# 666DZY666/micronet

Measured on NVIDIA H100. Metric: qat_step_images_per_sec, higher is better.
Workload: dtype f32 (bf16 tensor-core products of exact integer levels / exact bf16 pieces, fp32 accumulate)

## Files before the change

### include/micronet_b200.h

```cpp
#ifndef MICRONET_B200_H
#define MICRONET_B200_H

#include <stdint.h>

#ifdef __cplusplus
extern "C" {
#endif

typedef void* mnb_stream_t;

#define MNB_E_ARG (-1)
#define MNB_E_UNSUPPORTED (-2)

int mnb_version(void);
const char* mnb_last_error(void);
int64_t mnb_launch_count(void);

typedef struct {
  int32_t batch, in_c, in_h, in_w;
  int32_t out_c, ker_h, ker_w;
  int32_t stride_h, stride_w, pad_h, pad_w, dil_h, dil_w, groups;
} mnb_conv_shape;

#define MNB_ACT_DOREFA 1
#define MNB_ACT_IAO 2
#define MNB_ACT_SIGN 3

typedef struct {
  int32_t mode;
  int32_t bits;
  int32_t qmin, qmax;
  int32_t q_type;
  const float* scale;
  const float* zero_point;
  const float* obs_min;
  const float* obs_max;
} mnb_act_qparams;

int mnb_act_quant_fwd(const float* x, int64_t n, const mnb_act_qparams* qp, uint8_t* codes,
                      uint32_t* pass_bits, float* xq, mnb_stream_t stream);
int mnb_act_quant_bwd(const float* g, const uint32_t* pass_bits, int64_t n, const mnb_act_qparams* qp,
                      float* dx, mnb_stream_t stream);

int mnb_bn_fold_fwd(const float* w, int32_t out_c, int32_t per_channel, const float* gamma, const float* beta,
                    const float* bias, const float* mean, const float* var, double eps, float* w_fused, float* b_fused,
                    mnb_stream_t stream);
int mnb_bn_fold_bwd(const float* dw_fused, const float* db_fused, const float* w, int32_t out_c, int32_t per_channel,
                    const float* gamma, const float* bias, const float* mean, const float* var, double eps, float* dw,
                    float* out6, mnb_stream_t stream);
int mnb_bn_fold_running(float* running_mean, float* running_var, const float* batch_mean, const float* batch_var, int32_t n,
                        double momentum, int32_t first, mnb_stream_t stream);

int mnb_quant_add_fwd(const float* a, const float* b, int64_t n, const mnb_act_qparams* qp, float* out,
                      uint32_t* pass_bits_a, uint32_t* pass_bits_b, int32_t relu ,
                      mnb_stream_t stream);
int mnb_quant_add_bwd(const float* g, const uint32_t* pass_bits_a, const uint32_t* pass_bits_b, int64_t n,
                      const mnb_act_qparams* qp, float* da, float* db, mnb_stream_t stream);

int64_t mnb_observe_scratch_bytes(int64_t n, int32_t rows);
int mnb_iao_observe(const float* x, int64_t n, int32_t rows, int32_t observer_kind, int32_t first,
                    double momentum, double percentile, float* min_val, float* max_val,
                    int32_t update_qparams, int32_t symmetric, int32_t qmin, int32_t qmax,
                    float* scale, float* zero_point, void* scratch, mnb_stream_t stream);
int mnb_iao_update_qparams(const float* min_val, const float* max_val, int32_t rows, int32_t symmetric,
                           int32_t qmin, int32_t qmax, float* scale, float* zero_point,
                           mnb_stream_t stream);

int mnb_dorefa_weight_fwd(const float* w, int64_t numel, int32_t out_c, int32_t w_bits, int16_t* w_int,
                          float* w_scale, float* wq, float* aux, void* scratch, mnb_stream_t stream);
int mnb_dorefa_weight_bwd(const float* g_wq, const float* aux, int64_t numel, int32_t w_bits, float* dw,
                          void* scratch, mnb_stream_t stream);
int mnb_wb_weight_fwd(float* w, int32_t out_c, int32_t in_c_per_group, int32_t ker_hw, int32_t W,
                      int16_t* w_int, float* w_scale, float* wq, float* aux, mnb_stream_t stream);
int mnb_wb_weight_bwd(const float* g_wq, const float* w, const float* aux, int32_t out_c,
                      int32_t in_c_per_group, int32_t ker_hw, int32_t W, float* dw, mnb_stream_t stream);
int mnb_iao_weight_fwd(const float* w, int64_t numel, int32_t out_c, int32_t rows, const float* scale,
                       const float* zero_point, const float* obs_min, const float* obs_max,
                       int32_t q_type, int32_t qmin, int32_t qmax, int16_t* w_int, float* w_scale,
                       float* wq, uint8_t* pass, mnb_stream_t stream);
int mnb_iao_weight_bwd(const float* g_wq, const uint8_t* pass, const float* scale, int64_t numel,
                       int32_t out_c, int32_t rows, float* dw, mnb_stream_t stream);

typedef struct {
  const uint8_t* a_codes;
  const float* a_f32;
  int32_t a_offset;
  const float* a_offset_zp;
  const float* a_scale;
  const int16_t* w_int;
  const float* w_scale;
  const float* w_f32;
  const float* bias;
} mnb_conv_operands;

int mnb_conv2d_fwd(const mnb_conv_shape* s, const mnb_conv_operands* op, float* y, mnb_stream_t stream);
int mnb_conv2d_dgrad(const mnb_conv_shape* s, const float* dy, const float* wq, const uint32_t* pass_bits,
                     const mnb_act_qparams* qp, float* dx, mnb_stream_t stream);
int64_t mnb_wgrad_scratch_bytes(const mnb_conv_shape* s);
int mnb_conv2d_wgrad(const mnb_conv_shape* s, const float* dy, const mnb_conv_operands* op, float* dwq,
                     void* scratch, mnb_stream_t stream);
int mnb_channel_stats(const float* x, int32_t batch, int32_t channels, int32_t hw, int32_t as_mean_var,
                      float* stats, void* scratch, mnb_stream_t stream);
int mnb_channel_stats_bwd(const float* x, const float* mean, const float* dmean, const float* dvar,
                          int32_t batch, int32_t channels, int32_t hw, float* dx, mnb_stream_t stream);

int mnb_fq_conv2d_fwd_tc(const mnb_conv_shape* s, const float* x, const mnb_act_qparams* qp,
                         const int16_t* w_int, const float* w_scale, const float* bias, float* y,
                         uint8_t* codes, uint32_t* pass_bits, void* wpack_scratch, int32_t* err_flag,
                         mnb_stream_t stream);

int mnb_conv2d_dgrad_tc(const mnb_conv_shape* s, const float* dy, const int16_t* w_int, const float* w_scale,
                        const uint32_t* pass_bits, const mnb_act_qparams* qp, float* dx, void* wpack_scratch,
                        int32_t* err_flag, mnb_stream_t stream);

int64_t mnb_wgrad_tc_scratch_bytes(const mnb_conv_shape* s);
int mnb_conv2d_wgrad_tc(const mnb_conv_shape* s, const float* dy, const float* x, const mnb_act_qparams* qp,
                        float* dwq, void* scratch, int32_t* inexact_flag, int32_t* err_flag, mnb_stream_t stream);
int mnb_conv2d_wgrad_cond(const mnb_conv_shape* s, const float* dy, const mnb_conv_operands* op, float* dwq,
                          void* scratch, const int32_t* run_if_nonzero, mnb_stream_t stream);

int mnb_bn_batch_stats(const float* x, int32_t batch, int32_t channels, int32_t hw, double eps, double momentum,
                       float* running_mean, float* running_var, int64_t* num_batches_tracked, float* mean_invstd,
                       void* scratch, mnb_stream_t stream);
int mnb_bn_sign_fwd(const float* x, int32_t batch, int32_t channels, int32_t hw, const float* mean, const float* invstd,
                    const float* gamma, const float* beta, int32_t out_shuffle_groups, float* y, uint32_t* pass_bits,
                    mnb_stream_t stream);
int mnb_bn_sign_bwd(const float* g, const uint32_t* pass_bits, const float* x, int32_t batch, int32_t channels, int32_t hw,
                    const float* mean, const float* invstd, const float* gamma, int32_t training,
                    int32_t out_shuffle_groups, float* dx, float* dgamma, float* dbeta, float* dx_channel_sum,
                    void* scratch, mnb_stream_t stream);

int mnb_bn_sign_pool_fwd(const float* x, int32_t batch, int32_t channels, int32_t H, int32_t W, const float* mean,
                         const float* invstd, const float* gamma, const float* beta, int32_t out_shuffle_groups, float* y,
                         uint32_t* pass_bits, uint8_t* argmax, mnb_stream_t stream);
int mnb_bn_sign_pool_bwd(const float* g, const uint32_t* pass_bits, const uint8_t* argmax, const float* x, int32_t batch,
                         int32_t channels, int32_t H, int32_t W, const float* mean, const float* invstd, const float* gamma,
                         int32_t training, int32_t out_shuffle_groups, float* dx, float* dgamma, float* dbeta,
                         float* dx_channel_sum, void* scratch, mnb_stream_t stream);

int mnb_maxpool2d_fwd(const float* x, int32_t batch, int32_t channels, int32_t H, int32_t W, int32_t kernel, int32_t stride,
                      int32_t pad, int32_t out_shuffle_groups, float* y, uint8_t* argmax, mnb_stream_t stream);
int mnb_maxpool2d_bwd(const float* g, const uint8_t* argmax, int32_t batch, int32_t channels, int32_t H, int32_t W,
                      int32_t kernel, int32_t stride, int32_t pad, int32_t out_shuffle_groups, float* dx,
                      mnb_stream_t stream);

int mnb_bn_sign_fwd_packed(const float* x, int32_t batch, int32_t channels, int32_t hw, const float* mean,
                           const float* invstd, const float* gamma, const float* beta, int32_t out_shuffle_groups, float* y,
                           uint32_t* pass_bits, void* x_packed, mnb_stream_t stream);

int mnb_fconv2d_fwd_tc(const mnb_conv_shape* s, const float* x, const float* w, const float* bias, float* y,
                       int32_t* err_flag, mnb_stream_t stream);
int64_t mnb_fconv2d_wgrad_tc_scratch_bytes(const mnb_conv_shape* s);
int mnb_fconv2d_wgrad_tc(const mnb_conv_shape* s, const float* dy, const float* x, float* dw, void* scratch,
                         int32_t* err_flag, mnb_stream_t stream);

int64_t mnb_pk_act_bytes(int32_t batch, int32_t channels, int32_t h, int32_t w, int32_t terms);
int mnb_pk_pack_act(const float* x, int32_t batch, int32_t channels, int32_t h, int32_t w, const mnb_act_qparams* qp,
                    int32_t terms, const float* ch_scale, int32_t phase_split, void* out_pk, uint8_t* bits8,
                    mnb_stream_t stream);
int mnb_bn_relu_quant_pack_fwd(const float* x, int32_t batch, int32_t channels, int32_t hw, const float* mean,
                               const float* invstd, const float* gamma, const float* beta, const mnb_act_qparams* qp,
                               int32_t out_shuffle_groups, void* x_packed, uint32_t* pass_bits, mnb_stream_t stream);
int mnb_bn_sign_bwd_pack(const float* g, const uint32_t* pass_bits, const float* x, int32_t batch, int32_t channels, int32_t hw,
                         const float* mean, const float* invstd, const float* gamma, const float* dgamma, const float* dbeta,
                         int32_t out_shuffle_groups, const float* ch_scale, int32_t terms, float* dx, void* dy_packed,
                         mnb_stream_t stream);
int mnb_bn_sign_pool_bwd_pack(const float* g, const uint32_t* pass_bits, const uint8_t* argmax, const float* x, int32_t batch,
                              int32_t channels, int32_t H, int32_t W, const float* mean, const float* invstd,
                              const float* gamma, const float* dgamma, const float* dbeta, int32_t out_shuffle_groups,
                              const float* ch_scale, int32_t terms, void* dy_packed, mnb_stream_t stream);
int mnb_pk_conv_codes(const mnb_conv_shape* s, const void* a_pk, int32_t terms_a, const void* w_img, int32_t terms_w,
                      const float* n_scale, const float* a_scale, float a_scale_const, const float* bias, int32_t level_bound,
                      int16_t* codes, float* dec, int32_t* err_flag, mnb_stream_t stream);
int mnb_codes_decode(const int16_t* codes, const float* dec, int32_t batch, int32_t channels, int32_t hw, float* x,
                     mnb_stream_t stream);
int mnb_bn_batch_stats_codes(const int16_t* codes, const float* dec, int32_t batch, int32_t channels, int32_t hw, double eps,
                             double momentum, float* running_mean, float* running_var, int64_t* num_batches_tracked,
                             float* mean_invstd, void* scratch, mnb_stream_t stream);
int mnb_bn_sign_fwd_packed_codes(const int16_t* codes, const float* dec, int32_t batch, int32_t channels, int32_t hw,
                                 const float* mean, const float* invstd, const float* gamma, const float* beta,
                                 int32_t out_shuffle_groups, float* y, uint32_t* pass_bits, void* x_packed, mnb_stream_t stream);
int mnb_bn_sign_bwd_codes(const float* g, const uint32_t* pass_bits, const int16_t* codes, const float* dec, int32_t batch,
                          int32_t channels, int32_t hw, const float* mean, const float* invstd, const float* gamma,
                          int32_t training, int32_t out_shuffle_groups, float* dx, float* dgamma, float* dbeta,
                          float* dx_channel_sum, void* scratch, mnb_stream_t stream);
int mnb_bn_sign_pool_fwd_codes(const int16_t* codes, const float* dec, int32_t batch, int32_t channels, int32_t H, int32_t W,
                               const float* mean, const float* invstd, const float* gamma, const float* beta,
                               int32_t out_shuffle_groups, float* y, uint32_t* pass_bits, uint8_t* argmax, mnb_stream_t stream);
int mnb_bn_sign_pool_bwd_codes(const float* g, const uint32_t* pass_bits, const uint8_t* argmax, const int16_t* codes,
                               const float* dec, int32_t batch, int32_t channels, int32_t H, int32_t W, const float* mean,
                               const float* invstd, const float* gamma, int32_t training, int32_t out_shuffle_groups, float* dx,
                               float* dgamma, float* dbeta, float* dx_channel_sum, void* scratch, mnb_stream_t stream);
int mnb_bn_sign_bwd_pack_codes(const float* g, const uint32_t* pass_bits, const int16_t* codes, const float* dec, int32_t batch,
                               int32_t channels, int32_t hw, const float* mean, const float* invstd, const float* gamma,
                               const float* dgamma, const float* dbeta, int32_t out_shuffle_groups, const float* ch_scale,
                               int32_t terms, float* dx, void* dy_packed, mnb_stream_t stream);
int mnb_bn_sign_pool_bwd_pack_codes(const float* g, const uint32_t* pass_bits, const uint8_t* argmax, const int16_t* codes,
                                    const float* dec, int32_t batch, int32_t channels, int32_t H, int32_t W, const float* mean,
                                    const float* invstd, const float* gamma, const float* dgamma, const float* dbeta,
                                    int32_t out_shuffle_groups, const float* ch_scale, int32_t terms, void* dy_packed,
                                    mnb_stream_t stream);
int mnb_pk_pack_act_relu(const float* x, int32_t batch, int32_t channels, int32_t h, int32_t w, const mnb_act_qparams* qp,
                         int32_t terms, const float* ch_scale, int32_t phase_split, int32_t relu, void* out_pk,
                         uint8_t* bits8, mnb_stream_t stream);
int mnb_pk_conv_plan(const mnb_conv_shape* s, int32_t mode, int32_t terms_a, int32_t terms_w, int32_t* out16);
int mnb_pk_conv_plan_ex(const mnb_conv_shape* s, int32_t mode, int32_t terms_a, int32_t terms_w, int32_t* out, int32_t n);
int mnb_pk_wgrad_plan(const mnb_conv_shape* s, int32_t terms_dy, int32_t terms_x, int32_t* out, int32_t n);
int64_t mnb_pk_wimage_bytes(const mnb_conv_shape* s, int32_t mode, int32_t terms_a, int32_t terms_w);
int mnb_pk_pack_weight(const mnb_conv_shape* s, int32_t mode, int32_t terms_a, int32_t terms_w, const int16_t* w_int,
                       const float* w_f32, const float* kzero, void* w_img, mnb_stream_t stream);
int mnb_pk_conv(const mnb_conv_shape* s, int32_t mode, const void* a_pk, int32_t terms_a, const void* w_img, int32_t terms_w,
                const float* n_scale, const float* a_scale, float a_scale_const, const float* bias, const uint8_t* bits8,
                float gain, float* out, int32_t* err_flag, mnb_stream_t stream);
typedef struct mnb_pk_post {
  const mnb_act_qparams* q;
  int32_t relu;
  int32_t phase_split;
  void* out_pk;
} mnb_pk_post;
int mnb_pk_conv_post(const mnb_conv_shape* s, const void* a_pk, int32_t terms_a, const void* w_img, int32_t terms_w,
                     const float* n_scale, const float* a_scale, float a_scale_const, const float* bias, float* out,
                     const mnb_pk_post* post, int32_t* err_flag, mnb_stream_t stream);
int mnb_quant_add_pack_fwd(const float* a, const float* b, int32_t batch, int32_t channels, int32_t h, int32_t w,
                           const mnb_act_qparams* qp, int32_t relu, float* out, const mnb_pk_post* post, mnb_stream_t stream);
int64_t mnb_pk_i8_act_bytes(int32_t batch, int32_t channels, int32_t h, int32_t w);
int mnb_pk_i8_pack_act(const float* x, int32_t batch, int32_t channels, int32_t h, int32_t w, const mnb_act_qparams* qp,
                       int32_t phase_split, int32_t relu, void* out_pk, mnb_stream_t stream);
int mnb_pk_i8_conv_plan(const mnb_conv_shape* s, int32_t* out, int32_t n);
int64_t mnb_pk_i8_wimage_bytes(const mnb_conv_shape* s);
int mnb_pk_i8_pack_weight(const mnb_conv_shape* s, const int16_t* w_int, void* w_img, mnb_stream_t stream);
int mnb_pk_i8_conv(const mnb_conv_shape* s, const void* a_pk, const void* w_img, const float* n_scale, const float* a_scale,
                   float a_scale_const, const float* bias, float* out, const mnb_pk_post* post, int32_t* err_flag,
                   mnb_stream_t stream);
int mnb_quant_add_pack_i8_fwd(const float* a, const float* b, int32_t batch, int32_t channels, int32_t h, int32_t w,
                              const mnb_act_qparams* qp, int32_t relu, float* out, const mnb_pk_post* post, mnb_stream_t stream);
int64_t mnb_pk_wgrad_scratch_bytes(const mnb_conv_shape* s, int32_t terms_dy, int32_t terms_x);
int mnb_pk_wgrad(const mnb_conv_shape* s, const void* dy_pk, int32_t terms_dy, const void* x_pk, int32_t terms_x,
                 const float* a_scale, const float* kdiv, float* dw, void* scratch, int32_t* err_flag, mnb_stream_t stream);
int mnb_pk_wgrad_taps_plan(const mnb_conv_shape* s, int32_t terms_dy, int32_t terms_x, int32_t* out, int32_t n);
int mnb_pk_wgrad_taps(const mnb_conv_shape* s, const void* dy_pk, int32_t terms_dy, const void* x_pk, int32_t terms_x,
                      const float* a_scale, const float* kdiv, float* dw, void* scratch, int32_t* err_flag, mnb_stream_t stream);

int mnb_xnor_supported(const mnb_conv_shape* s);
int64_t mnb_xnor_act_bytes(int32_t batch, int32_t channels, int32_t h, int32_t w, int32_t groups);
int mnb_xnor_pack_act(const float* x, int32_t batch, int32_t channels, int32_t h, int32_t w, int32_t groups, void* out_bits,
                      mnb_stream_t stream);
int64_t mnb_xnor_wimage_bytes(const mnb_conv_shape* s);
int mnb_xnor_pack_weight(const mnb_conv_shape* s, const int16_t* w_int, void* w_img, mnb_stream_t stream);
int mnb_xnor_conv_fwd(const mnb_conv_shape* s, const void* a_bits, const void* w_img, const float* alpha, const float* bias,
                      float* y, mnb_stream_t stream);

int mnb_adam_step(float* params, const float* grads, float* exp_avg, float* exp_avg_sq, int64_t n, float lr,
                  float beta1, float beta2, float eps, float weight_decay, int32_t step, mnb_stream_t stream);

void mnb_set_tc_profile_buffer(void* dev_int64x16);

int mnb_selftest_umma(const float* A, const float* B, float* D, int32_t N, int32_t K, int32_t int8,
                      int32_t* err_flag, mnb_stream_t stream);
int mnb_selftest_tma3d(const float* src, const int64_t* dims3_host, const int32_t* box3_host,
                       const int32_t* coord3_host, float* out, int32_t* err_flag, mnb_stream_t stream);

int mnb_selftest_mma_rate(int32_t N, int32_t n_acc, int32_t a_shift16, int32_t iters, int32_t mn_major,
                          int64_t* out2, int32_t* err_flag, mnb_stream_t stream);

#ifdef __cplusplus
}
#endif
#endif
```

### micronet_b200/_lib.py

```python
from __future__ import annotations

import ctypes as C
import os

import torch

_HERE = os.path.dirname(os.path.abspath(__file__))
LIB_PATH = os.path.join(_HERE, "lib", "libmicronet_b200.so")

ACT_DOREFA, ACT_IAO, ACT_SIGN = 1, 2, 3


class ConvShape(C.Structure):
    _fields_ = [(n, C.c_int32) for n in (
        "batch", "in_c", "in_h", "in_w", "out_c", "ker_h", "ker_w", "stride_h", "stride_w",
        "pad_h", "pad_w", "dil_h", "dil_w", "groups")]


class ActQParams(C.Structure):
    _fields_ = [("mode", C.c_int32), ("bits", C.c_int32), ("qmin", C.c_int32), ("qmax", C.c_int32),
                ("q_type", C.c_int32), ("scale", C.c_void_p), ("zero_point", C.c_void_p),
                ("obs_min", C.c_void_p), ("obs_max", C.c_void_p)]


class PkPost(C.Structure):
    _fields_ = [("q", C.POINTER(ActQParams)), ("relu", C.c_int32), ("phase_split", C.c_int32), ("out_pk", C.c_void_p)]


class ConvOperands(C.Structure):
    _fields_ = [("a_codes", C.c_void_p), ("a_f32", C.c_void_p), ("a_offset", C.c_int32),
                ("a_offset_zp", C.c_void_p), ("a_scale", C.c_void_p), ("w_int", C.c_void_p),
                ("w_scale", C.c_void_p), ("w_f32", C.c_void_p), ("bias", C.c_void_p)]


_P, _I, _L, _D = C.c_void_p, C.c_int32, C.c_int64, C.c_double
_SHAPE, _ACTQ, _OPS = C.POINTER(ConvShape), C.POINTER(ActQParams), C.POINTER(ConvOperands)

PROTOTYPES = {
    "mnb_version": (C.c_int, []),
    "mnb_last_error": (C.c_char_p, []),
    "mnb_launch_count": (_L, []),
    "mnb_act_quant_fwd": (C.c_int, [_P, _L, _ACTQ, _P, _P, _P, _P]),
    "mnb_act_quant_bwd": (C.c_int, [_P, _P, _L, _ACTQ, _P, _P]),
    "mnb_bn_fold_fwd": (C.c_int, [_P, _I, _I, _P, _P, _P, _P, _P, _D, _P, _P, _P]),
    "mnb_bn_fold_bwd": (C.c_int, [_P, _P, _P, _I, _I, _P, _P, _P, _P, _D, _P, _P, _P]),
    "mnb_bn_fold_running": (C.c_int, [_P, _P, _P, _P, _I, _D, _I, _P]),
    "mnb_quant_add_fwd": (C.c_int, [_P, _P, _L, _ACTQ, _P, _P, _P, _I, _P]),
    "mnb_quant_add_bwd": (C.c_int, [_P, _P, _P, _L, _ACTQ, _P, _P, _P]),
    "mnb_observe_scratch_bytes": (_L, [_L, _I]),
    "mnb_iao_observe": (C.c_int, [_P, _L, _I, _I, _I, _D, _D, _P, _P, _I, _I, _I, _I, _P, _P, _P, _P]),
    "mnb_iao_update_qparams": (C.c_int, [_P, _P, _I, _I, _I, _I, _P, _P, _P]),
    "mnb_dorefa_weight_fwd": (C.c_int, [_P, _L, _I, _I, _P, _P, _P, _P, _P, _P]),
    "mnb_dorefa_weight_bwd": (C.c_int, [_P, _P, _L, _I, _P, _P, _P]),
    "mnb_wb_weight_fwd": (C.c_int, [_P, _I, _I, _I, _I, _P, _P, _P, _P, _P]),
    "mnb_wb_weight_bwd": (C.c_int, [_P, _P, _P, _I, _I, _I, _I, _P, _P]),
    "mnb_iao_weight_fwd": (C.c_int, [_P, _L, _I, _I, _P, _P, _P, _P, _I, _I, _I, _P, _P, _P, _P, _P]),
    "mnb_iao_weight_bwd": (C.c_int, [_P, _P, _P, _L, _I, _I, _P, _P]),
    "mnb_conv2d_fwd": (C.c_int, [_SHAPE, _OPS, _P, _P]),
    "mnb_conv2d_dgrad": (C.c_int, [_SHAPE, _P, _P, _P, _ACTQ, _P, _P]),
    "mnb_wgrad_scratch_bytes": (_L, [_SHAPE]),
    "mnb_conv2d_wgrad": (C.c_int, [_SHAPE, _P, _OPS, _P, _P, _P]),
    "mnb_channel_stats": (C.c_int, [_P, _I, _I, _I, _I, _P, _P, _P]),
    "mnb_channel_stats_bwd": (C.c_int, [_P, _P, _P, _P, _I, _I, _I, _P, _P]),
    "mnb_fq_conv2d_fwd_tc": (C.c_int, [_SHAPE, _P, _ACTQ, _P, _P, _P, _P, _P, _P, _P, _P, _P]),
    "mnb_conv2d_dgrad_tc": (C.c_int, [_SHAPE, _P, _P, _P, _P, _ACTQ, _P, _P, _P, _P]),
    "mnb_wgrad_tc_scratch_bytes": (_L, [_SHAPE]),
    "mnb_conv2d_wgrad_tc": (C.c_int, [_SHAPE, _P, _P, _ACTQ, _P, _P, _P, _P, _P]),
    "mnb_conv2d_wgrad_cond": (C.c_int, [_SHAPE, _P, _OPS, _P, _P, _P, _P]),
    "mnb_bn_batch_stats": (C.c_int, [_P, _I, _I, _I, _D, _D, _P, _P, _P, _P, _P, _P]),
    "mnb_bn_sign_fwd": (C.c_int, [_P, _I, _I, _I, _P, _P, _P, _P, _I, _P, _P, _P]),
    "mnb_bn_sign_bwd": (C.c_int, [_P, _P, _P, _I, _I, _I, _P, _P, _P, _I, _I, _P, _P, _P, _P, _P, _P]),
    "mnb_bn_sign_pool_fwd": (C.c_int, [_P, _I, _I, _I, _I, _P, _P, _P, _P, _I, _P, _P, _P, _P]),
    "mnb_bn_sign_pool_bwd": (C.c_int, [_P, _P, _P, _P, _I, _I, _I, _I, _P, _P, _P, _I, _I, _P, _P, _P, _P, _P, _P]),
    "mnb_bn_sign_fwd_packed": (C.c_int, [_P, _I, _I, _I, _P, _P, _P, _P, _I, _P, _P, _P, _P]),
    "mnb_fconv2d_fwd_tc": (C.c_int, [_SHAPE, _P, _P, _P, _P, _P, _P]),
    "mnb_fconv2d_wgrad_tc_scratch_bytes": (_L, [_SHAPE]),
    "mnb_fconv2d_wgrad_tc": (C.c_int, [_SHAPE, _P, _P, _P, _P, _P, _P]),
    "mnb_maxpool2d_fwd": (C.c_int, [_P, _I, _I, _I, _I, _I, _I, _I, _I, _P, _P, _P]),
    "mnb_maxpool2d_bwd": (C.c_int, [_P, _P, _I, _I, _I, _I, _I, _I, _I, _I, _P, _P]),
    "mnb_adam_step": (C.c_int, [_P, _P, _P, _P, _L, C.c_float, C.c_float, C.c_float, C.c_float, C.c_float, _I, _P]),
    "mnb_pk_act_bytes": (_L, [_I, _I, _I, _I, _I]),
    "mnb_pk_pack_act": (C.c_int, [_P, _I, _I, _I, _I, _ACTQ, _I, _P, _I, _P, _P, _P]),
    "mnb_bn_relu_quant_pack_fwd": (C.c_int, [_P, _I, _I, _I, _P, _P, _P, _P, _ACTQ, _I, _P, _P, _P]),
    "mnb_pk_pack_act_relu": (C.c_int, [_P, _I, _I, _I, _I, _ACTQ, _I, _P, _I, _I, _P, _P, _P]),
    "mnb_pk_conv_plan": (C.c_int, [_SHAPE, _I, _I, _I, _P]),
    "mnb_pk_conv_plan_ex": (C.c_int, [_SHAPE, _I, _I, _I, _P, _I]),
    "mnb_pk_wgrad_plan": (C.c_int, [_SHAPE, _I, _I, _P, _I]),
    "mnb_pk_wimage_bytes": (_L, [_SHAPE, _I, _I, _I]),
    "mnb_pk_pack_weight": (C.c_int, [_SHAPE, _I, _I, _I, _P, _P, _P, _P, _P]),
    "mnb_pk_conv": (C.c_int, [_SHAPE, _I, _P, _I, _P, _I, _P, _P, C.c_float, _P, _P, C.c_float, _P, _P, _P]),
    "mnb_bn_sign_bwd_pack": (C.c_int, [_P, _P, _P, _I, _I, _I, _P, _P, _P, _P, _P, _I, _P, _I, _P, _P, _P]),
    "mnb_bn_sign_pool_bwd_pack": (C.c_int, [_P, _P, _P, _P, _I, _I, _I, _I, _P, _P, _P, _P, _P, _I, _P, _I, _P, _P]),
    "mnb_pk_conv_post": (C.c_int, [_SHAPE, _P, _I, _P, _I, _P, _P, C.c_float, _P, _P, C.POINTER(PkPost), _P, _P]),
    "mnb_pk_conv_codes": (C.c_int, [_SHAPE, _P, _I, _P, _I, _P, _P, C.c_float, _P, _I, _P, _P, _P, _P]),
    "mnb_codes_decode": (C.c_int, [_P, _P, _I, _I, _I, _P, _P]),
    "mnb_bn_batch_stats_codes": (C.c_int, [_P, _P, _I, _I, _I, _D, _D, _P, _P, _P, _P, _P, _P]),
    "mnb_bn_sign_fwd_packed_codes": (C.c_int, [_P, _P, _I, _I, _I, _P, _P, _P, _P, _I, _P, _P, _P, _P]),
    "mnb_bn_sign_bwd_codes": (C.c_int, [_P, _P, _P, _P, _I, _I, _I, _P, _P, _P, _I, _I, _P, _P, _P, _P, _P, _P]),
    "mnb_bn_sign_pool_fwd_codes": (C.c_int, [_P, _P, _I, _I, _I, _I, _P, _P, _P, _P, _I, _P, _P, _P, _P]),
    "mnb_bn_sign_pool_bwd_codes": (C.c_int, [_P, _P, _P, _P, _P, _I, _I, _I, _I, _P, _P, _P, _I, _I, _P, _P, _P, _P, _P, _P]),
    "mnb_bn_sign_bwd_pack_codes": (C.c_int, [_P, _P, _P, _P, _I, _I, _I, _P, _P, _P, _P, _P, _I, _P, _I, _P, _P, _P]),
    "mnb_bn_sign_pool_bwd_pack_codes": (C.c_int, [_P, _P, _P, _P, _P, _I, _I, _I, _I, _P, _P, _P, _P, _P, _I, _P, _I, _P,
                                                  _P]),
    "mnb_quant_add_pack_fwd": (C.c_int, [_P, _P, _I, _I, _I, _I, _ACTQ, _I, _P, C.POINTER(PkPost), _P]),
    "mnb_pk_i8_act_bytes": (_L, [_I, _I, _I, _I]),
    "mnb_pk_i8_pack_act": (C.c_int, [_P, _I, _I, _I, _I, _ACTQ, _I, _I, _P, _P]),
    "mnb_pk_i8_conv_plan": (C.c_int, [_SHAPE, _P, _I]),
    "mnb_pk_i8_wimage_bytes": (_L, [_SHAPE]),
    "mnb_pk_i8_pack_weight": (C.c_int, [_SHAPE, _P, _P, _P]),
    "mnb_pk_i8_conv": (C.c_int, [_SHAPE, _P, _P, _P, _P, C.c_float, _P, _P, C.POINTER(PkPost), _P, _P]),
    "mnb_quant_add_pack_i8_fwd": (C.c_int, [_P, _P, _I, _I, _I, _I, _ACTQ, _I, _P, C.POINTER(PkPost), _P]),
    "mnb_pk_wgrad_scratch_bytes": (_L, [_SHAPE, _I, _I]),
    "mnb_pk_wgrad": (C.c_int, [_SHAPE, _P, _I, _P, _I, _P, _P, _P, _P, _P, _P]),
    "mnb_pk_wgrad_taps_plan": (C.c_int, [_SHAPE, _I, _I, _P, _I]),
    "mnb_pk_wgrad_taps": (C.c_int, [_SHAPE, _P, _I, _P, _I, _P, _P, _P, _P, _P, _P]),
    "mnb_xnor_supported": (C.c_int, [_SHAPE]),
    "mnb_xnor_act_bytes": (_L, [_I, _I, _I, _I, _I]),
    "mnb_xnor_pack_act": (C.c_int, [_P, _I, _I, _I, _I, _I, _P, _P]),
    "mnb_xnor_wimage_bytes": (_L, [_SHAPE]),
    "mnb_xnor_pack_weight": (C.c_int, [_SHAPE, _P, _P, _P]),
    "mnb_xnor_conv_fwd": (C.c_int, [_SHAPE, _P, _P, _P, _P, _P, _P]),
    "mnb_set_tc_profile_buffer": (None, [_P]),
    "mnb_selftest_mma_rate": (C.c_int, [_I, _I, _I, _I, _I, _P, _P, _P]),
    "mnb_selftest_umma": (C.c_int, [_P, _P, _P, _I, _I, _I, _P, _P]),
    "mnb_selftest_tma3d": (C.c_int, [_P, C.POINTER(C.c_int64), C.POINTER(C.c_int32), C.POINTER(C.c_int32), _P, _P, _P]),
}

_lib = None


def load():
    global _lib
    if _lib is not None:
        return _lib
    if not os.path.exists(LIB_PATH):
        raise RuntimeError(
            f"micronet_b200: {LIB_PATH} is missing - build it with `python -m micronet_b200.build` "
            "(there is no CPU / PyTorch fallback for the fake-quant hot path)")
    lib = C.CDLL(LIB_PATH)
    for name, (res, args) in PROTOTYPES.items():
        fn = getattr(lib, name)
        fn.restype, fn.argtypes = res, args
    _lib = lib
    return lib


def check(rc: int, what: str):
    if rc != 0:
        msg = load().mnb_last_error().decode(errors="replace")
        kind = ValueError if rc < 0 else RuntimeError
        raise kind(f"micronet_b200.{what} failed (code {rc}): {msg}")


def ptr(t):
    return None if t is None else t.data_ptr()


def stream():
    return torch.cuda.current_stream().cuda_stream


def require_cuda(*tensors):
    for t in tensors:
        if t is not None and not t.is_cuda:
            raise RuntimeError(
                "micronet_b200: the fake-quant engine runs on CUDA (sm_90a) tensors only; "
                "got a CPU tensor - there is deliberately no CPU fallback")


def require_f32(*tensors):
    for t in tensors:
        if t is not None and t.dtype != torch.float32:
            raise TypeError(f"micronet_b200: fp32 tensors only (the reference's QAT modules are fp32), got {t.dtype}")


def launch_count() -> int:
    return int(load().mnb_launch_count())


_errflags = {}


def tc_err_flag(device):
    key = (device.type, device.index)
    if key not in _errflags:
        _errflags[key] = torch.zeros(1, dtype=torch.int32, device=device)
    return _errflags[key]


def tc_check(device=None):
    for key, flag in _errflags.items():
        code = int(flag.item())
        if code:
            raise RuntimeError(f"micronet_b200: tensor-core pipeline wait timed out (code {code}) on {key}")


E_UNSUPPORTED = -2
KEEP_DEBUG = False
USE_TC = os.environ.get("MNB_DISABLE_TC", "0") != "1"
USE_PACKED = os.environ.get("MNB_PACKED_OPERANDS", "0") == "1"
PK_MODE = os.environ.get("MNB_PK", "auto")
PK_TERMS = int(os.environ.get("MNB_PK_TERMS", "3"))
PK_TERMS_BWD = int(os.environ.get("MNB_PK_TERMS_BWD", "2"))
PK_WBWTAB = os.environ.get("MNB_PK_WBWTAB", "1") == "1"
PK_WG_TAPS = os.environ.get("MNB_PK_WG_TAPS", "1") != "0"

XNOR_MODE = os.environ.get("MNB_XNOR", "auto")

PLANE_ONLY = os.environ.get("MNB_PLANE_ONLY", "1") == "1"

_scratch = {}


def scratch(device, rows=1):
    lib = load()
    need = int(lib.mnb_observe_scratch_bytes(0, int(rows)))
    key = (device.type, device.index)
    buf = _scratch.get(key)
    if buf is None or buf.numel() < need:
        buf = torch.zeros(max(need, 1 << 20), dtype=torch.uint8, device=device)
        _scratch[key] = buf
    return buf
```

### micronet_b200/csrc/mnb_pk.cu

```cuda
#include <cuda.h>
#include <cuda_bf16.h>

#include <algorithm>
#include <cstdlib>
#include <cstring>

#include "mnb_common.cuh"
#include "mnb_tc.cuh"

namespace pk {

constexpr int MAXST = 8;
constexpr int MAXTAP = 64, MAXTMPL = 16, MAXY = 4, MAXPAIR = 6, MAXPROG = 512;
constexpr int kSmemBudget = 227 * 1024 - 3072;
constexpr int kNtSizes[] = {16, 32, 48, 64, 96, 128};

struct Tmpl { int kph, tap0, ntap, blk_off, blk_bytes; };

struct Plan {
  int mode;
  int B, G, R, S, stride;
  int HA, WA, C8A, nkph;
  int kg, ng, NOUT;
  int OHr, OWr, OH, OW, omul, ny;
  int hlo, hhi, wlo, whi;
  int Wt, BW, TH, THH, TB, npos, col_tiles, row_tiles, img_tiles, n_mtiles;
  int Nt, n_ntiles, MT, n_mgroups, n_items;
  int CC, ksteps, chunks;
  int TA, TBk, npairs, pair_a[MAXPAIR], pair_b[MAXPAIR];
  int ntmpl[MAXY], ntap[MAXY];
  Tmpl tmpl[MAXY][MAXTMPL];
  int tap_aoff[MAXY][MAXTAP];
  short tap_r[MAXY][MAXTAP], tap_s[MAXY][MAXTAP];
  int img_bytes[MAXY], y_off[MAXY];
  int64_t wimg_bytes;
  int a_box_bytes, a_bytes, b_off, stage_bytes, nstage, st_log2, smem_bytes, off_stg;
  int segmented, seg_len;
  int cpu;
};

static inline int ceil_div(int a, int b) { return (a + b - 1) / b; }
static inline int round_up(int a, int b) { return ceil_div(a, b) * b; }

static void make_pairs(int TA, int TBk, Plan& p) {
  const int lim = std::max(TA, TBk) - 1;
  p.npairs = 0;
  for (int sum = lim; sum >= 0; --sum)
    for (int a = 0; a < TA; ++a) {
      const int b = sum - a;
      if (b < 0 || b >= TBk) continue;
      if (p.npairs < MAXPAIR) { p.pair_a[p.npairs] = a; p.pair_b[p.npairs] = b; ++p.npairs; }
    }
}

static int unsupported(const char* why) { return mnb_fail(MNB_E_UNSUPPORTED, "pk conv: %s", why); }

static int make_plan(const mnb_conv_shape* s, int mode, int TA, int TBk, Plan& p, int cpu = 8) {
  MNB_REQUIRE(s != nullptr, "conv shape is NULL");
  memset(&p, 0, sizeof(p));
  const int C = s->in_c, K = s->out_c, G = s->groups, H = s->in_h, W = s->in_w, R = s->ker_h, S = s->ker_w;
  MNB_REQUIRE(s->batch > 0 && C > 0 && K > 0 && H > 0 && W > 0 && G > 0 && C % G == 0 && K % G == 0 && R > 0 && S > 0,
              "bad conv shape");
  MNB_REQUIRE(TA >= 1 && TA <= 3 && TBk >= 1 && TBk <= 3, "term counts must be 1..3");
  MNB_REQUIRE(cpu == 8 || (cpu == 16 && mode == 0 && TA == 1 && TBk == 1), "int8 plans are single-product forward plans");
  if (s->dil_h != 1 || s->dil_w != 1) return unsupported("dilation != 1");
  if (s->stride_h != s->stride_w || (s->stride_h != 1 && s->stride_h != 2)) return unsupported("stride must be 1 or 2");
  const int st = s->stride_h, ph_ = s->pad_h, pw_ = s->pad_w;
  if (ph_ > R - 1 || pw_ > S - 1) return unsupported("padding larger than the filter");
  const int P = (H + 2 * ph_ - R) / st + 1, Q = (W + 2 * pw_ - S) / st + 1;
  if (P < 1 || Q < 1) return unsupported("empty output");
  if (st == 2 && ((H | W) & 1)) return unsupported("stride 2 needs even H and W");
  const int cin_g = C / G, cout_g = K / G;
  p.mode = mode; p.B = s->batch; p.G = G; p.R = R; p.S = S; p.stride = st;
  p.TA = TA; p.TBk = TBk; p.cpu = cpu;
  make_pairs(TA, TBk, p);
  if (mode == 0) {
    p.kg = cin_g; p.ng = cout_g; p.NOUT = K;
    p.nkph = st == 2 ? 4 : 1;
    p.HA = H / st; p.WA = W / st; p.C8A = ceil_div(C, cpu);
    p.OHr = P; p.OWr = Q; p.OH = P; p.OW = Q; p.omul = 1; p.ny = 1;
  } else {
    p.kg = cout_g; p.ng = cin_g; p.NOUT = C;
    p.nkph = 1; p.HA = P; p.WA = Q; p.C8A = ceil_div(K, 8);
    p.OHr = H / st; p.OWr = W / st; p.OH = H; p.OW = W; p.omul = st; p.ny = st == 2 ? 4 : 1;
  }
  if (G > 1 && (p.kg % cpu))
    return unsupported(cpu == 8 ? "grouped conv needs GEMM-K channels per group % 8 == 0"
                                : "grouped int8 conv needs GEMM-K channels per group % 16 == 0");
  if (cpu == 16 && (int64_t)p.kg * R * S * 128 * 127 > (int64_t)INT32_MAX) return unsupported("int8 sums could overflow s32");
  struct Tap { int kph, sh, sw, r, s; };
  Tap taps[MAXY][MAXTAP];
  int hlo = 0, hhi = 0, wlo = 0, whi = 0;
  for (int y = 0; y < p.ny; ++y) {
    int n = 0;
    const int ya = y >> 1, yb = y & 1;
    for (int kph = 0; kph < p.nkph; ++kph)
      for (int r = 0; r < R; ++r)
        for (int q = 0; q < S; ++q) {
          int kp = 0, sh, sw;
          if (mode == 0) {
            const int dr = r - ph_, ds = q - pw_;
            if (st == 1) { sh = dr; sw = ds; }
            else {
              const int fh = dr & 1, fw = ds & 1;
              kp = fh * 2 + fw; sh = (dr - fh) / 2; sw = (ds - fw) / 2;
            }
          } else {
            if (st == 1) { sh = ph_ - r; sw = pw_ - q; }
            else {
              const int th = ya + ph_ - r, tw = yb + pw_ - q;
              if ((th & 1) || (tw & 1)) continue;
              sh = th / 2; sw = tw / 2;
            }
          }
          if (kp != kph) continue;
          if (n >= MAXTAP) return unsupported("more than 64 filter taps");
          taps[y][n++] = Tap{kph, sh, sw, r, q};
          hlo = std::max(hlo, -sh); hhi = std::max(hhi, sh); wlo = std::max(wlo, -sw); whi = std::max(whi, sw);
        }
    p.ntap[y] = n;
  }
  p.hlo = hlo; p.hhi = hhi; p.wlo = wlo; p.whi = whi;
  const int halo_w = wlo + whi;
  if (halo_w >= 96) return unsupported("filter too wide");
  {
    const int ct_min = ceil_div(p.OWr, 128 - halo_w);
    double best = 1e30;
    int ct_max = std::min(p.OWr, ct_min + 14);
    if (p.npairs > 1) {
      const int wt0 = ceil_div(p.OWr, ct_min), bw0 = wt0 + halo_w;
      const int th0 = std::max(1, std::min(p.OHr, (128 - wt0) / bw0 + 1));
      if ((double)((th0 + hlo + hhi) * bw0) / (double)(th0 * wt0) <= 2.2) ct_max = ct_min;
    }
    for (int ct = ct_min; ct <= ct_max; ++ct) {
      const int wt = ceil_div(p.OWr, ct), bw = wt + halo_w;
      if (ceil_div(p.OWr, wt) != ct) continue;
      const int th = std::max(1, std::min(p.OHr, (128 - wt) / bw + 1));
      const double amp = (double)((th + hlo + hhi) * bw) / (double)(th * wt);
      const double cost = (double)ct * ceil_div(p.OHr, th) * (1.0 + 0.25 * amp) * (1.0 + 3.2 / wt);
      if (cost < best - 1e-9) { best = cost; p.col_tiles = ct; p.Wt = wt; p.BW = bw; p.TH = th; }
    }
    if (const char* e = getenv("MNB_PK_COLTILES")) {
      const int ct = atoi(e);
      if (ct >= ct_min && ct <= p.OWr) {
        p.col_tiles = ct; p.Wt = ceil_div(p.OWr, ct); p.col_tiles = ceil_div(p.OWr, p.Wt); p.BW = p.Wt + halo_w;
        p.TH = std::max(1, std::min(p.OHr, (128 - p.Wt) / p.BW + 1));
      }
    }
  }
  p.THH = p.TH + hlo + hhi;
  p.TB = 1;
  if (p.TH == p.OHr && p.col_tiles == 1) {
    const int last = (p.TH - 1) * p.BW + p.Wt;
    p.TB = std::max(1, std::min(p.B, (128 - last) / (p.THH * p.BW) + 1));
  }
  if (p.BW > 128 || p.THH > 256 || p.TB > 256) return unsupported("box dimension");
  p.npos = p.TB * p.THH * p.BW;
  p.row_tiles = ceil_div(p.OHr, p.TH);
  p.img_tiles = ceil_div(p.B, p.TB);
  p.n_mtiles = p.img_tiles * p.row_tiles * p.col_tiles;
  const int ng16 = round_up(p.ng, 16);
  {
    int seg_target = 64;
    if (const char* e = getenv("MNB_PK_SEG_MMAS")) seg_target = std::max(1, atoi(e));
    int chain = 0;
    for (int y = 0; y < p.ny; ++y) chain = std::max(chain, p.ntap[y] * p.npairs * ceil_div(p.kg, 16));
    p.segmented = p.npairs > 1 && chain > seg_target;
  }
  {
    const int ntiles = ceil_div(ng16, 128);
    const int want = round_up(ceil_div(ng16, ntiles), 16);
    p.Nt = 128;
    for (int v : kNtSizes) if (v >= want) { p.Nt = v; break; }
  }
  p.n_ntiles = ceil_div(p.ng, p.Nt);
  p.MT = 1;
  {
    auto wave_eff = [&](int mt) {
      const int64_t items = (int64_t)ceil_div(p.n_mtiles, mt) * p.n_ntiles * G;
      const int64_t ctas = std::max<int64_t>(1, MNB_NUM_SMS / p.ny);
      return (double)items / (double)(ceil_div((int)std::min<int64_t>(items, 1 << 30), (int)ctas) * ctas);
    };
    const int cap = std::max(1, 128 / p.Nt);
    for (int mt = 2; mt <= std::min(4, cap); mt *= 2) {
      if (p.n_mtiles < mt) break;
      if ((int64_t)ceil_div(p.n_mtiles, mt) * p.n_ntiles * G * p.ny < 120) break;
      if (wave_eff(mt) >= wave_eff(1) - 0.04) p.MT = mt;
    }
  }
  if (const char* e = getenv("MNB_PK_MT")) {
    const int v = atoi(e);
    if ((v == 1 || v == 2 || v == 4) && v * p.Nt <= 128) p.MT = v;
  }
  p.n_mgroups = ceil_div(p.n_mtiles, p.MT);
  p.n_items = p.n_mgroups * p.n_ntiles * G;
  const int nk16 = ceil_div(p.kg, 2 * cpu);
  int maxtap_kph = 1;
  for (int y = 0; y < p.ny; ++y)
    for (int i = 0, run = 0; i < p.ntap[y]; ++i) {
      run = (i > 0 && taps[y][i].kph == taps[y][i - 1].kph) ? run + 1 : 1;
      maxtap_kph = std::max(maxtap_kph, run);
    }
  const int a16 = p.MT * TA * round_up(2 * p.npos * 16, 128);
  auto b16 = [&](int tg) { return TBk * tg * 2 * p.Nt * 16; };
  const int stage_target = 56 * 1024;
  int TG = std::min(maxtap_kph, 25);
  while (TG > 1 && a16 + b16(TG) > stage_target) --TG;
  if (a16 + b16(TG) > (kSmemBudget - 8192) / 2) return unsupported("one 16-channel stage does not fit in shared memory");
  int cc16 = std::max(1, std::min(nk16, stage_target / (a16 + b16(TG))));
  cc16 = std::min(cc16, 16);
  p.chunks = ceil_div(nk16, cc16);
  cc16 = ceil_div(nk16, p.chunks);
  p.CC = cc16 * 2 * cpu; p.ksteps = cc16;
  p.a_box_bytes = (p.CC / cpu) * p.npos * 16;
  p.a_bytes = round_up(p.a_box_bytes, 128);
  p.b_off = p.MT * TA * p.a_bytes;
  int64_t total = 0;
  int max_blk = 0;
  for (int y = 0; y < p.ny; ++y) {
    int nt = 0, off = 0;
    for (int i = 0; i < p.ntap[y];) {
      int j = i;
      while (j < p.ntap[y] && taps[y][j].kph == taps[y][i].kph && j - i < TG) ++j;
      if (nt >= MAXTMPL) return unsupported("too many tap groups");
      Tmpl& t = p.tmpl[y][nt++];
      t.kph = taps[y][i].kph; t.tap0 = i; t.ntap = j - i;
      t.blk_bytes = TBk * t.ntap * (p.CC / cpu) * p.Nt * 16;
      t.blk_off = off;
      off += p.chunks * t.blk_bytes;
      max_blk = std::max(max_blk, t.blk_bytes);
      i = j;
    }
    p.ntmpl[y] = nt;
    p.img_bytes[y] = off;
    p.y_off[y] = (int)total;
    total += (int64_t)off * p.n_ntiles * G;
    if (total > (int64_t)1 << 30) return unsupported("weight image larger than 1 GiB");
    for (int i = 0; i < p.ntap[y]; ++i) {
      p.tap_aoff[y][i] = (taps[y][i].sh + hlo) * p.BW + (taps[y][i].sw + wlo);
      p.tap_r[y][i] = (short)taps[y][i].r; p.tap_s[y][i] = (short)taps[y][i].s;
    }
  }
  p.wimg_bytes = std::max<int64_t>(total, 16);
  p.seg_len = 1 << 30;
  if (p.segmented) {
    const int per_stage = TG * p.npairs * p.ksteps;
    int target = 64;
    if (const char* e = getenv("MNB_PK_SEG_MMAS")) target = std::max(1, atoi(e));
    p.seg_len = std::max(1, target / per_stage);
  }
  p.stage_bytes = round_up(p.b_off + max_blk, 1024);
  const int slack = round_up((128 + (hlo + hhi) * p.BW + halo_w + 8) * 16, 1024);
  const int stg = 32 * tc::kStageLd * 4;
  int nst = (kSmemBudget - slack - stg) / p.stage_bytes;
  if (nst < 2) return unsupported("fewer than two pipeline stages fit");
  p.nstage = nst >= 8 ? 8 : (nst >= 4 ? 4 : 2);
  if (const char* e = getenv("MNB_PK_STAGES")) { const int v = atoi(e); if ((v == 2 || v == 4 || v == 8) && v <= nst) p.nstage = v; }
  p.st_log2 = p.nstage == 8 ? 3 : (p.nstage == 4 ? 2 : 1);
  p.off_stg = p.nstage * p.stage_bytes + slack;
  p.smem_bytes = p.off_stg + stg;
  if (p.MT * p.Nt > 128) return unsupported("accumulators exceed the register budget");
  return 0;
}

__device__ __forceinline__ uint32_t pack2(float a, float b) {
  __nv_bfloat162 v = __floats2bfloat162_rn(a, b);
  return *reinterpret_cast<uint32_t*>(&v);
}

__device__ __forceinline__ uint32_t pack4_s8(float a, float b, float c, float d) {
  return ((uint32_t)__float2int_rn(a) & 0xffu) | (((uint32_t)__float2int_rn(b) & 0xffu) << 8) |
         (((uint32_t)__float2int_rn(c) & 0xffu) << 16) | ((uint32_t)__float2int_rn(d) << 24);
}
__device__ __forceinline__ uint4 pack16_s8(const float (&l)[16]) {
  return make_uint4(pack4_s8(l[0], l[1], l[2], l[3]), pack4_s8(l[4], l[5], l[6], l[7]), pack4_s8(l[8], l[9], l[10], l[11]),
                    pack4_s8(l[12], l[13], l[14], l[15]));
}

template <int QUANT>
__global__ void __launch_bounds__(256) pack_act_kernel(const float* __restrict__ x, int B, int C, int H, int W, int C8,
                                                       int terms, const float* __restrict__ ch_scale, mnb_act_qparams qp,
                                                       int a_off, int phase_split, uint4* __restrict__ out,
                                                       int64_t plane_vecs, uint8_t* __restrict__ bits8, int relu) {
  MnbActQ q;
  float zp = 0.f;
  if (QUANT) {
    q = mnb_load_actq(qp);
    if (qp.mode == MNB_ACT_IAO && qp.zero_point) zp = __ldg(qp.zero_point);
  }
  const uint32_t HW = (uint32_t)H * (uint32_t)W;
  const uint32_t plane = blockIdx.y * blockDim.y + threadIdx.y;
  if (plane >= (uint32_t)B * (uint32_t)C8) return;
  const uint32_t b = plane / (uint32_t)C8, c8 = plane - b * (uint32_t)C8;
  for (uint32_t pos = blockIdx.x * blockDim.x + threadIdx.x; pos < HW; pos += gridDim.x * blockDim.x) {
    const int64_t idx = (int64_t)plane * HW + pos;
    float v[8];
    uint32_t passbits = 0;
    const float* src = x + ((int64_t)b * C + c8 * 8) * HW + pos;
#pragma unroll
    for (int j = 0; j < 8; ++j) {
      const int c = (int)c8 * 8 + j;
      float val = c < C ? __ldg(src + (int64_t)j * HW) : 0.f;
      if (relu) val = fmaxf(val, 0.f);
      if (!QUANT && ch_scale) val = c < C ? __fmul_rn(val, __ldg(ch_scale + c)) : 0.f;
      v[j] = val;
    }
    if (QUANT) {
      float lev[8];
      mnb_act_levels<8>(q, v, lev, passbits);
      uint32_t live = 0;
#pragma unroll
      for (int j = 0; j < 8; ++j) {
        const bool in = (int)c8 * 8 + j < C;
        v[j] = in ? lev[j] + zp : 0.f;
        live |= in ? (1u << j) : 0u;
      }
      passbits &= live;
    }
    int64_t dst;
    if (phase_split) {
      const uint32_t h = pos / (uint32_t)W, w = pos - h * (uint32_t)W;
      const uint32_t oct = ((h & 1u) * 2u + (w & 1u)) * (uint32_t)C8 + c8;
      dst = (((int64_t)b * 4 * C8 + oct) * (H >> 1) + (h >> 1)) * (W >> 1) + (w >> 1);
    } else {
      dst = idx;
    }
    for (int tm = 0; tm < terms; ++tm) {
      uint32_t pk4[4];
#pragma unroll
      for (int j = 0; j < 4; ++j) {
        pk4[j] = pack2(v[2 * j], v[2 * j + 1]);
        v[2 * j] -= __uint_as_float(pk4[j] << 16);
        v[2 * j + 1] -= __uint_as_float(pk4[j] & 0xffff0000u);
      }
      out[(int64_t)tm * plane_vecs + dst] = make_uint4(pk4[0], pk4[1], pk4[2], pk4[3]);
    }
    if (QUANT && bits8) bits8[idx] = (uint8_t)passbits;
  }
}

__global__ void __launch_bounds__(256) pack_act_i8_kernel(const float* __restrict__ x, int B, int C, int H, int W, int C16,
                                                          mnb_act_qparams qp, int phase_split, int relu, uint4* __restrict__ out) {
  const MnbActQ q = mnb_load_actq(qp);
  const float zp = qp.zero_point ? __ldg(qp.zero_point) : 0.f;
  const uint32_t HW = (uint32_t)H * (uint32_t)W;
  const uint32_t plane = blockIdx.y * blockDim.y + threadIdx.y;
  if (plane >= (uint32_t)B * (uint32_t)C16) return;
  const uint32_t b = plane / (uint32_t)C16, c16 = plane - b * (uint32_t)C16;
  for (uint32_t pos = blockIdx.x * blockDim.x + threadIdx.x; pos < HW; pos += gridDim.x * blockDim.x) {
    const float* src = x + ((int64_t)b * C + c16 * 16) * HW + pos;
    float v[16], lev[16];
#pragma unroll
    for (int j = 0; j < 16; ++j) {
      float val = (int)c16 * 16 + j < C ? __ldg(src + (int64_t)j * HW) : 0.f;
      if (relu) val = fmaxf(val, 0.f);
      v[j] = val;
    }
    uint32_t passbits;
    mnb_act_levels<16>(q, v, lev, passbits);
#pragma unroll
    for (int j = 0; j < 16; ++j) lev[j] = (int)c16 * 16 + j < C ? lev[j] + zp : 0.f;
    int64_t dst;
    if (phase_split) {
      const uint32_t h = pos / (uint32_t)W, w = pos - h * (uint32_t)W;
      const uint32_t u = ((h & 1u) * 2u + (w & 1u)) * (uint32_t)C16 + c16;
      dst = (((int64_t)b * 4 * C16 + u) * (H >> 1) + (h >> 1)) * (W >> 1) + (w >> 1);
    } else {
      dst = (int64_t)plane * HW + pos;
    }
    out[dst] = pack16_s8(lev);
  }
}

__global__ void __launch_bounds__(256) bn_relu_quant_pack_kernel(const float* __restrict__ x, int batch, int channels, int hw,
                                                                 int sg, const float* __restrict__ mean,
                                                                 const float* __restrict__ invstd, const float* __restrict__ gamma,
                                                                 const float* __restrict__ beta, mnb_act_qparams qp,
                                                                 uint32_t* __restrict__ bits, uint4* __restrict__ xp) {
  const int lane = threadIdx.x & 31;
  const int c8n = channels / 8, p32n = hw / 32, cpg = channels / sg;
  const int64_t items = (int64_t)batch * c8n * p32n;
  const int64_t nwarps = ((int64_t)gridDim.x * blockDim.x) >> 5;
  const MnbActQ q = mnb_load_actq(qp);
  for (int64_t w = ((int64_t)blockIdx.x * blockDim.x + threadIdx.x) >> 5; w < items; w += nwarps) {
    const int p32 = (int)(w % p32n);
    const int64_t t = w / p32n;
    const int oc8 = (int)(t % c8n), b = (int)(t / c8n);
    const int pos = p32 * 32 + lane;
    float lev[8], yv[8], bnv[8];
#pragma unroll
    for (int j = 0; j < 8; ++j) {
      const int oc = oc8 * 8 + j;
      const int c = sg > 1 ? (oc % sg) * cpg + oc / sg : oc;
      const int64_t fi = ((int64_t)b * channels + c) * hw + pos;
      bnv[j] = fmaf(__ldg(x + fi) - __ldg(mean + c), __ldg(gamma + c) * __ldg(invstd + c), __ldg(beta + c));
      yv[j] = fmaxf(bnv[j], 0.f);
    }
    uint32_t passbits;
    mnb_act_levels<8>(q, yv, lev, passbits);
#pragma unroll
    for (int j = 0; j < 8; ++j) {
      const int oc = oc8 * 8 + j;
      const int c = sg > 1 ? (oc % sg) * cpg + oc / sg : oc;
      const int64_t fi = ((int64_t)b * channels + c) * hw + pos;
      const uint32_t word = __ballot_sync(0xffffffffu, ((passbits >> j) & 1u) && bnv[j] > 0.f);
      if (lane == 0) bits[fi >> 5] = word;
    }
    xp[((int64_t)b * c8n + oc8) * hw + pos] = make_uint4(pack2(lev[0], lev[1]), pack2(lev[2], lev[3]), pack2(lev[4], lev[5]),
                                                          pack2(lev[6], lev[7]));
  }
}

template <int CPU>
__global__ void __launch_bounds__(256) quant_add_pack_kernel(const float* __restrict__ a, const float* __restrict__ b, int B, int C,
// ... 419 lines not shown
#pragma unroll
            for (int mt = 0; mt < MAXMT; ++mt) {
              if (mt >= (int)p.m.MT) break;
              const uint32_t a_base = a_lo0 + s16 + (uint32_t)mt * p.m.a_mt16, b_base = b_lo0 + s16;
              for (uint32_t e = 0; e < pc; ++e) {
                const uint4 w4 = p.m.prog4[pb + e];
                const uint32_t w[4] = {w4.x, w4.y, w4.z, w4.w};
#pragma unroll
                for (int k = 0; k < 4; ++k) {
                  if (w[k] == 0xffffffffu) continue;
                  if constexpr (I8)
                    tc::Mma<NT>::s8(reinterpret_cast<int32_t(&)[NR]>(acc[mt]), a_hi | (uint64_t)(a_base + (w[k] & 0xffffu)),
                                    b_hi | (uint64_t)(b_base + (w[k] >> 16)), 1);
                  else
                    tc::Mma<NT>::template bf16<0, 0>(acc[mt], a_hi | (uint64_t)(a_base + (w[k] & 0xffffu)),
                                                      b_hi | (uint64_t)(b_base + (w[k] >> 16)), 1);
                }
              }
            }
          }
          tc::wg_commit();
          tc::wg_wait<0>();
#pragma unroll
          for (int mt = 0; mt < MAXMT; ++mt) tc::fence_acc(acc[mt]);
          __syncwarp();
          if (lane == 0) tc::mbar_arrive(&sh.empty[slot]);
          if (SEG && ++seg_pos == p.m.seg_len) {
            seg_pos = 0;
#pragma unroll
            for (int mt = 0; mt < MAXMT; ++mt) {
#pragma unroll
              for (int i = 0; i < NR; ++i) { rs[SEG ? mt : 0][SEG ? i : 0] = __fadd_rn(rs[SEG ? mt : 0][SEG ? i : 0], acc[mt][i]); acc[mt][i] = 0.f; }
            }
          }
        }
      }
      if (SEG) {
#pragma unroll
        for (int mt = 0; mt < MAXMT; ++mt) {
#pragma unroll
          for (int i = 0; i < NR; ++i) rs[SEG ? mt : 0][SEG ? i : 0] = __fadd_rn(rs[SEG ? mt : 0][SEG ? i : 0], acc[mt][i]);
        }
      }
      if constexpr (I8) {
#pragma unroll
        for (int mt = 0; mt < MAXMT; ++mt) {
#pragma unroll
          for (int i = 0; i < NR; ++i) acc[mt][i] = __int2float_rn(__float_as_int(acc[mt][i]));
        }
      }
      int mt_cur = -1;
      bool valid = false;
      int64_t orow = 0;
      const uint8_t* brow = nullptr;
      int64_t prow = 0;
      auto do_slot = [&](const int mt, const int c16, const float (&r)[16]) {
        const int n0 = c16 * 16;
        if (mt != mt_cur) {
          mt_cur = mt;
          const int tile = mg * p.MT + mt;
          uint32_t ct_u, r2_u, rt_u, bt_u;
          e_ct.divmod((uint32_t)tile, r2_u, ct_u);
          e_rt.divmod(r2_u, bt_u, rt_u);
          const int ct = (int)ct_u, rt = (int)rt_u, bt = (int)bt_u;
          const int b = bt * p.TB + tb, i = rt * p.TH + th, j = ct * p.Wt + wc;
          valid = row_ok && tile < p.n_mtiles && b < p.B && i < p.OHr && j < p.OWr;
          const int oh = i * p.omul + ya, ow = j * p.omul + yb;
          orow = ((int64_t)b * p.NOUT + n_base) * plane + (int64_t)oh * p.OW + ow;
          brow = p.bits8 ? p.bits8 + (int64_t)b * p.C8O * plane + (int64_t)oh * p.OW + ow : nullptr;
          if (p.post_out) {
            if (p.post_split)
              prow = (((int64_t)b * 4 * p.C8O + ((oh & 1) * 2 + (ow & 1)) * p.C8O) * (p.OH >> 1) + (oh >> 1)) * (p.OW >> 1) + (ow >> 1);
            else
              prow = ((int64_t)b * p.C8O * p.OH + oh) * p.OW + ow;
          }
        }
        if (!valid || n0 >= n_cnt || (p.dbg & 1)) return;
        if (!SEG && !I8 && p.codes) {
          int16_t* cp = p.codes + orow + (int64_t)n0 * plane;
#pragma unroll
          for (int k = 0; k < 16; ++k, cp += plane)
            if (n0 + k < n_cnt) *cp = (int16_t)__float2int_rn(r[k]);
          return;
        }
        float sc[16], bs[16];
#pragma unroll
        for (int v = 0; v < 4; ++v) {
          const float4 a = *reinterpret_cast<const float4*>(&sh.epi_scale[n0 + 4 * v]);
          const float4 c = *reinterpret_cast<const float4*>(&sh.epi_bias[n0 + 4 * v]);
          sc[4 * v] = a.x; sc[4 * v + 1] = a.y; sc[4 * v + 2] = a.z; sc[4 * v + 3] = a.w;
          bs[4 * v] = c.x; bs[4 * v + 1] = c.y; bs[4 * v + 2] = c.z; bs[4 * v + 3] = c.w;
        }
        float* op = p.out + orow + (int64_t)n0 * plane;
        if (!SEG && p.post_out) {
          float lev[16], yv[16];
#pragma unroll
          for (int k = 0; k < 16; ++k) {
            const float v = fmaf(r[k], sc[k], bs[k]);
            if (p.out && n0 + k < n_cnt) op[(int64_t)k * plane] = v;
            yv[k] = p.post_relu ? fmaxf(v, 0.f) : v;
          }
          uint32_t passbits;
          mnb_act_levels<16>(pq, yv, lev, passbits);
#pragma unroll
          for (int k = 0; k < 16; ++k) lev[k] = n0 + k < n_cnt ? lev[k] + pzp : 0.f;
          const int64_t oct_stride = p.post_split ? (int64_t)(p.OH >> 1) * (p.OW >> 1) : plane;
          if constexpr (I8) {
            p.post_out[prow + (int64_t)((n_base + n0) >> 4) * oct_stride] = pack16_s8(lev);
          } else {
            const int oc8 = (n_base + n0) >> 3;
            uint4* dst = p.post_out + prow + (int64_t)oc8 * oct_stride;
            dst[0] = make_uint4(pack2(lev[0], lev[1]), pack2(lev[2], lev[3]), pack2(lev[4], lev[5]), pack2(lev[6], lev[7]));
            if (n0 + 8 < n_cnt)
              dst[oct_stride] = make_uint4(pack2(lev[8], lev[9]), pack2(lev[10], lev[11]), pack2(lev[12], lev[13]), pack2(lev[14], lev[15]));
          }
        } else if (p.mode == 0 || !brow) {
#pragma unroll
          for (int k = 0; k < 16; ++k, op += plane)
            if (n0 + k < n_cnt) *op = fmaf(r[k], sc[k], bs[k]);
        } else {
          const int oc0 = (n_base + n0) >> 3;
          const uint32_t m0 = __ldg(brow + (int64_t)oc0 * plane);
          const uint32_t m1 = (n0 + 8 < n_cnt) ? __ldg(brow + (int64_t)(oc0 + 1) * plane) : 0u;
          const uint32_t mask = m0 | (m1 << 8);
#pragma unroll
          for (int k = 0; k < 16; ++k, op += plane)
            if (n0 + k < n_cnt) *op = ((mask >> k) & 1u) ? r[k] * p.gain : 0.f;
        }
      };
      const int ncols = (int)p.m.MT * NT;
#pragma unroll
      for (int rnd = 0; rnd < (MAXMT * NT + 31) / 32; ++rnd) {
        if (32 * rnd >= ncols) break;
        epi_bar_sync<NEPI>();
#pragma unroll
        for (int mt = 0; mt < MAXMT; ++mt) {
          const int lo = mt * NT > 32 * rnd ? mt * NT : 32 * rnd;
          const int hi = (mt + 1) * NT < 32 * rnd + 32 ? (mt + 1) * NT : 32 * rnd + 32;
          if (lo >= hi) continue;
          float* dst = stage + (lo - 32 * rnd) * tc::kStageLd;
          if constexpr (SEG) tc::frag_cols_to_smem(rs[mt], dst, tc::kStageLd, 64 * wg, lo - mt * NT, hi - lo);
          else tc::frag_cols_to_smem(acc[mt], dst, tc::kStageLd, 64 * wg, lo - mt * NT, hi - lo);
        }
        epi_bar_sync<NEPI>();
        const int L0 = 32 * rnd + 16 * half;
        if (L0 < ncols) {
          float r[16];
#pragma unroll
          for (int k = 0; k < 16; ++k) r[k] = stage[(16 * half + k) * tc::kStageLd + m];
          do_slot(L0 / NT, (L0 % NT) >> 4, r);
        }
      }
      epi_bar_sync<NEPI>();
    }
  }
done:
  __syncthreads();
}

static int make_pk_tmap(CUtensorMap* m, const void* base, int64_t plane_bytes, int t, int B, int C8tot, int H, int W,
                        int bw, int bh, int bb, int bc8) {
  const uint64_t HW = (uint64_t)H * W;
  uint64_t dims[4] = {(uint64_t)W * 2, (uint64_t)H, (uint64_t)B, (uint64_t)C8tot};
  uint64_t strides[3] = {(uint64_t)W * 16, (uint64_t)C8tot * HW * 16, HW * 16};
  uint32_t box[4] = {(uint32_t)bw * 2, (uint32_t)bh, (uint32_t)bb, (uint32_t)bc8};
  return mnb_make_tmap_strided(m, reinterpret_cast<const uint8_t*>(base) + (int64_t)t * plane_bytes, 8, 4, dims, strides, box);
}

template <typename K>
static int set_max_smem(K kernel, int bytes) {
  static const void* seen_fn[32];
  static int seen_dev[32], nseen = 0;
  int dev = 0;
  cudaGetDevice(&dev);
  const void* fn = reinterpret_cast<const void*>(kernel);
  for (int i = 0; i < nseen; ++i)
    if (seen_fn[i] == fn && seen_dev[i] == dev) return 0;
  cudaError_t ce = cudaFuncSetAttribute(kernel, cudaFuncAttributeMaxDynamicSharedMemorySize, bytes);
  if (ce != cudaSuccess) return mnb_fail((int)ce, "cudaFuncSetAttribute: %s", cudaGetErrorString(ce));
  if (nseen < 32) { seen_fn[nseen] = fn; seen_dev[nseen] = dev; ++nseen; }
  return 0;
}

struct WgPlan {
  int B, G, R, S, stride, ntap;
  int P, Q, K8, HX, WX, C8X, nkph;
  int cin_g, cout_g, gm;
  int hlo, hhi, wlo, whi, BW, TH, THH, rows_dy, rows_x, row_tiles;
  int Nc, n_ctiles, n_ktiles, tpg, n_tg, NI, nsub, nstg_total, splits, stg_per_split;
  int TA, TX, npairs, pair_a[MAXPAIR], pair_b[MAXPAIR];
  int tap_kph[MAXTAP], tap_off[MAXTAP];
  int kph_used[4], nkph_used, kph_slot[4];
  int dy_box_bytes, x_box_bytes, dy_bytes, x_bytes, sub_bytes, stage_bytes, nstage, st_log2, smem_bytes;
  int64_t partial_floats;
};

static int make_wg_plan_nc(const mnb_conv_shape* s, int TA, int TX, WgPlan& p, int nc_cap) {
  MNB_REQUIRE(s != nullptr, "conv shape is NULL");
  memset(&p, 0, sizeof(p));
  const int C = s->in_c, K = s->out_c, G = s->groups, H = s->in_h, W = s->in_w, R = s->ker_h, S = s->ker_w;
  MNB_REQUIRE(s->batch > 0 && C > 0 && K > 0 && H > 0 && W > 0 && G > 0 && C % G == 0 && K % G == 0, "bad conv shape");
  if (s->dil_h != 1 || s->dil_w != 1) return mnb_fail(MNB_E_UNSUPPORTED, "pk wgrad: dilation != 1");
  if (s->stride_h != s->stride_w || (s->stride_h != 1 && s->stride_h != 2)) return mnb_fail(MNB_E_UNSUPPORTED, "pk wgrad: stride");
  const int st = s->stride_h, ph_ = s->pad_h, pw_ = s->pad_w;
  if (ph_ > R - 1 || pw_ > S - 1) return mnb_fail(MNB_E_UNSUPPORTED, "pk wgrad: padding larger than the filter");
  if (st == 2 && ((H | W) & 1)) return mnb_fail(MNB_E_UNSUPPORTED, "pk wgrad: stride 2 needs even H and W");
  if (R * S > MAXTAP) return mnb_fail(MNB_E_UNSUPPORTED, "pk wgrad: more than 64 taps");
  p.B = s->batch; p.G = G; p.R = R; p.S = S; p.stride = st; p.ntap = R * S;
  p.P = (H + 2 * ph_ - R) / st + 1; p.Q = (W + 2 * pw_ - S) / st + 1;
  if (p.P < 1 || p.Q < 1) return mnb_fail(MNB_E_UNSUPPORTED, "pk wgrad: empty output");
  p.cin_g = C / G; p.cout_g = K / G;
  if (G > 1 && ((p.cin_g % 8) || (p.cout_g % 8))) return mnb_fail(MNB_E_UNSUPPORTED, "pk wgrad: grouped conv needs channels per group % 8 == 0");
  p.gm = 1;
  while (G % (p.gm * 2) == 0 && p.gm * 2 * p.cout_g <= 128 && p.gm * 2 * p.cin_g <= 128) p.gm *= 2;
  if (const char* e = getenv("MNB_PK_WG_MERGE")) { if (atoi(e) == 0) p.gm = 1; }
  p.G = G / p.gm; p.cin_g *= p.gm; p.cout_g *= p.gm;
  p.K8 = ceil_div(K, 8); p.C8X = ceil_div(C, 8);
  p.nkph = st == 2 ? 4 : 1; p.HX = H / st; p.WX = W / st;
  p.TA = TA; p.TX = TX;
  { Plan tmp; memset(&tmp, 0, sizeof(tmp)); make_pairs(TA, TX, tmp); p.npairs = tmp.npairs;
    for (int i = 0; i < tmp.npairs; ++i) { p.pair_a[i] = tmp.pair_a[i]; p.pair_b[i] = tmp.pair_b[i]; } }
  int sh_[MAXTAP], sw_[MAXTAP];
  int hlo = 0, hhi = 0, wlo = 0, whi = 0;
  for (int i = 0; i < 4; ++i) p.kph_slot[i] = -1;
  for (int r = 0; r < R; ++r)
    for (int q = 0; q < S; ++q) {
      const int t = r * S + q, dr = r - ph_, ds = q - pw_;
      int kp = 0, sh = dr, sw = ds;
      if (st == 2) { const int fh = dr & 1, fw = ds & 1; kp = fh * 2 + fw; sh = (dr - fh) / 2; sw = (ds - fw) / 2; }
      p.tap_kph[t] = kp; sh_[t] = sh; sw_[t] = sw;
      if (p.kph_slot[kp] < 0) { p.kph_slot[kp] = p.nkph_used; p.kph_used[p.nkph_used++] = kp; }
      hlo = std::max(hlo, -sh); hhi = std::max(hhi, sh); wlo = std::max(wlo, -sw); whi = std::max(whi, sw);
    }
  p.hlo = hlo; p.hhi = hhi; p.wlo = wlo; p.whi = whi;
  const int need = p.Q + wlo + whi;
  if (need > 128) return mnb_fail(MNB_E_UNSUPPORTED, "pk wgrad: row wider than 128 positions");
  int nc = std::min(nc_cap, round_up(p.cin_g, 16));
  if (const char* e = getenv("MNB_PK_WG_NC")) nc = std::max(16, std::min(nc, atoi(e) / 16 * 16));
  p.n_ctiles = ceil_div(p.cin_g, nc);
  p.Nc = round_up(ceil_div(p.cin_g, p.n_ctiles), 16);
  p.n_ctiles = ceil_div(p.cin_g, p.Nc);
  p.n_ktiles = ceil_div(p.cout_g, 128);
  p.tpg = std::max(1, std::min(p.ntap, 128 / p.Nc));
  p.n_tg = ceil_div(p.ntap, p.tpg);
  p.tpg = ceil_div(p.ntap, p.n_tg);
  if (p.tpg * p.Nc > 128) return mnb_fail(MNB_E_UNSUPPORTED, "pk wgrad: accumulators exceed the register budget");
  auto sub_bytes_of = [&](int bw, int th) {
    const int dyb = round_up(16 * th * bw * 16, 128);
    const int xb = round_up((p.Nc / 8) * (th + hlo + hhi) * bw * 16 + 16 * 16, 128);
    return TA * dyb + TX * p.nkph_used * xb;
  };
  int best_bw = 0, best_th = 0;
  double best_score = -1;
  for (int pass = 0; pass < 2 && !best_bw; ++pass) {
    const int limit = (kSmemBudget - 2048) / (pass == 0 ? 4 : 2);
    for (int bw = need; bw <= std::min(128, need + 15); ++bw)
      for (int th = 1; th <= p.P; ++th) {
        if ((th * bw) % 16) continue;
        if (th + hlo + hhi > 256 || sub_bytes_of(bw, th) > limit) continue;
        const double eff = (double)p.Q / bw, fill = std::min(1.0, (double)th * bw / 64.0);
        const double score = eff * (0.5 + 0.5 * fill);
        if (score > best_score) { best_score = score; best_bw = bw; best_th = th; }
      }
  }
  if (!best_bw) return mnb_fail(MNB_E_UNSUPPORTED, "pk wgrad: no raster fits shared memory (N tile %d)", p.Nc);
  p.BW = best_bw; p.TH = best_th; p.THH = p.TH + hlo + hhi;
  p.rows_dy = p.TH * p.BW; p.rows_x = p.THH * p.BW;
  p.row_tiles = ceil_div(p.P, p.TH);
  for (int t = 0; t < p.ntap; ++t) p.tap_off[t] = (sh_[t] + hlo) * p.BW + (sw_[t] + wlo);
  p.dy_box_bytes = 16 * p.rows_dy * 16;
  p.x_box_bytes = (p.Nc / 8) * p.rows_x * 16;
  p.dy_bytes = round_up(p.dy_box_bytes, 128);
  p.x_bytes = round_up(p.x_box_bytes + 16 * 16, 128);
  p.sub_bytes = TA * p.dy_bytes + TX * p.nkph_used * p.x_bytes;
  p.nsub = p.B * p.row_tiles;
  const int stage_target = 52 * 1024;
  p.NI = std::max(1, std::min(std::min(p.nsub, 8), stage_target / p.sub_bytes));
  p.stage_bytes = round_up(p.NI * p.sub_bytes, 1024);
  const int nst = (kSmemBudget - 1024) / p.stage_bytes;
  if (nst < 2) return mnb_fail(MNB_E_UNSUPPORTED, "pk wgrad: fewer than two stages fit");
  p.nstage = nst >= 4 ? 4 : 2;
  p.st_log2 = p.nstage == 4 ? 2 : 1;
  p.smem_bytes = p.nstage * p.stage_bytes + 1024;
  p.nstg_total = ceil_div(p.nsub, p.NI);
  const int n_kc = p.n_ktiles * p.n_ctiles * p.G * p.n_tg;
  p.splits = std::max(1, std::min(p.nstg_total, std::max(1, MNB_NUM_SMS / n_kc)));
  const int chain_per_stage = p.NI * (p.rows_dy / 16) * p.npairs;
  int chain_max = 256;
  if (const char* e = getenv("MNB_PK_WG_CHAIN")) chain_max = std::max(1, atoi(e));
  while (p.splits < p.nstg_total && (int64_t)ceil_div(p.nstg_total, p.splits) * chain_per_stage > chain_max) ++p.splits;
  p.stg_per_split = ceil_div(p.nstg_total, p.splits);
  p.splits = ceil_div(p.nstg_total, p.stg_per_split);
  p.partial_floats = (int64_t)p.splits * p.G * p.n_ktiles * p.n_ctiles * p.ntap * p.Nc * 128;
  return 0;
}

static int make_wg_plan(const mnb_conv_shape* s, int TA, int TX, WgPlan& p) {
  int rc = MNB_E_UNSUPPORTED;
  for (int cap = 128; cap >= 16; cap /= 2) {
    rc = make_wg_plan_nc(s, TA, TX, p, cap);
    if (rc != MNB_E_UNSUPPORTED) return rc;
  }
  return rc;
}

struct WgParams {
// ... 380 lines not shown
template <typename XT>
static int bn_sign_bwd_pack(const float* g, const uint32_t* pass_bits, const XT* x, const float* dec, int32_t batch,
                            int32_t channels, int32_t hw, const float* mean, const float* invstd, const float* gamma,
                            const float* dgamma, const float* dbeta, int32_t out_shuffle_groups, const float* ch_scale,
                            int32_t terms, float* dx, void* dy_packed, mnb_stream_t stream) {
  MNB_REQUIRE(g && pass_bits && x && mean && invstd && gamma && dgamma && dbeta && dy_packed, "NULL bn_sign_bwd_pack pointer");
  MNB_REQUIRE(batch > 0 && channels > 0 && hw > 0 && terms >= 1 && terms <= 3, "bad bn_sign_bwd_pack arguments");
  MNB_REQUIRE(out_shuffle_groups >= 1 && channels % out_shuffle_groups == 0, "shuffle groups %d do not divide %d channels",
              out_shuffle_groups, channels);
  if (channels % 8 || (reinterpret_cast<uintptr_t>(dy_packed) & 15))
    return mnb_fail(MNB_E_UNSUPPORTED, "packed BatchNorm backward needs channels %% 8 == 0 and a 16-byte aligned output");
  if (hw % 32) return mnb_fail(MNB_E_UNSUPPORTED, "packed BatchNorm backward needs H*W %% 32 == 0");
  const int c8n = channels / 8;
  auto al = [](const void* p, int a) { return p == nullptr || (reinterpret_cast<uintptr_t>(p) & (uintptr_t)(a - 1)) == 0; };
  constexpr int xs = (int)sizeof(XT);
  const int vec = (hw % 128 == 0 && al(g, 16) && al(x, 4 * xs) && al(dx, 16)) ? 4
                  : ((hw % 64 == 0 && al(g, 8) && al(x, 2 * xs) && al(dx, 8)) ? 2 : 1);
  const int64_t warps = (int64_t)batch * c8n * (hw / (32 * vec));
  const int blocks = (int)std::min<int64_t>(mnb_ceil_div(warps, 8), (int64_t)MNB_NUM_SMS * 8);
  const float inv_count = 1.f / (float)((int64_t)batch * hw);
  uint4* outp = reinterpret_cast<uint4*>(dy_packed);
  const int64_t plane_vecs = (int64_t)batch * c8n * hw;
  cudaStream_t st = (cudaStream_t)stream;
#define MNB_BWD_PACK(V)                                                                                                          \
  pk::bn_sign_bwd_pack_kernel<V, XT><<<blocks, 256, 0, st>>>(g, pass_bits, x, dec, batch, channels, hw, out_shuffle_groups,     \
                                                             inv_count, mean, invstd, gamma, dgamma, dbeta, ch_scale, terms, dx, \
                                                             outp, plane_vecs)
  if (vec == 4) MNB_BWD_PACK(4); else if (vec == 2) MNB_BWD_PACK(2); else MNB_BWD_PACK(1);
#undef MNB_BWD_PACK
  MNB_LAUNCHED(1);
  return 0;
}

extern "C" int mnb_bn_sign_bwd_pack(const float* g, const uint32_t* pass_bits, const float* x, int32_t batch, int32_t channels,
                                    int32_t hw, const float* mean, const float* invstd, const float* gamma, const float* dgamma,
                                    const float* dbeta, int32_t out_shuffle_groups, const float* ch_scale, int32_t terms,
                                    float* dx, void* dy_packed, mnb_stream_t stream) {
  return bn_sign_bwd_pack<float>(g, pass_bits, x, nullptr, batch, channels, hw, mean, invstd, gamma, dgamma, dbeta,
                                 out_shuffle_groups, ch_scale, terms, dx, dy_packed, stream);
}

extern "C" int mnb_bn_sign_bwd_pack_codes(const float* g, const uint32_t* pass_bits, const int16_t* codes, const float* dec,
                                          int32_t batch, int32_t channels, int32_t hw, const float* mean, const float* invstd,
                                          const float* gamma, const float* dgamma, const float* dbeta, int32_t out_shuffle_groups,
                                          const float* ch_scale, int32_t terms, float* dx, void* dy_packed, mnb_stream_t stream) {
  MNB_REQUIRE(dec, "NULL decode pair");
  return bn_sign_bwd_pack<int16_t>(g, pass_bits, codes, dec, batch, channels, hw, mean, invstd, gamma, dgamma, dbeta,
                                   out_shuffle_groups, ch_scale, terms, dx, dy_packed, stream);
}

template <typename XT>
static int bn_sign_pool_bwd_pack(const float* g, const uint32_t* pass_bits, const uint8_t* argmax, const XT* x, const float* dec,
                                 int32_t batch, int32_t channels, int32_t H, int32_t W, const float* mean, const float* invstd,
                                 const float* gamma, const float* dgamma, const float* dbeta, int32_t out_shuffle_groups,
                                 const float* ch_scale, int32_t terms, void* dy_packed, mnb_stream_t stream) {
  MNB_REQUIRE(g && pass_bits && argmax && x && mean && invstd && gamma && dgamma && dbeta && dy_packed, "NULL bn_sign_pool_bwd_pack pointer");
  MNB_REQUIRE(batch > 0 && channels > 0 && H > 0 && W > 0 && terms >= 1 && terms <= 3, "bad bn_sign_pool_bwd_pack arguments");
  MNB_REQUIRE(out_shuffle_groups >= 1 && channels % out_shuffle_groups == 0, "shuffle groups %d do not divide %d channels",
              out_shuffle_groups, channels);
  if ((H & 1) || (W & 7) || channels % 8 || (int64_t)batch * channels * H * W >= (1ll << 31) ||
      (reinterpret_cast<uintptr_t>(x) & (4 * sizeof(XT) - 1)) || (reinterpret_cast<uintptr_t>(dy_packed) & 15) ||
      (reinterpret_cast<uintptr_t>(g) & 7))
    return mnb_fail(MNB_E_UNSUPPORTED, "packed pooled BatchNorm backward needs even H, W %% 8 == 0, channels %% 8 == 0, aligned tensors");
  const int c8n = channels / 8;
  const int64_t total = (int64_t)batch * c8n * (H / 2) * (W / 4);
  const int blocks = (int)std::min<int64_t>(mnb_ceil_div(total, 256), (int64_t)MNB_NUM_SMS * 8);
  pk::bn_sign_pool_bwd_pack_kernel<XT><<<blocks, 256, 0, (cudaStream_t)stream>>>(
      reinterpret_cast<const float2*>(g), reinterpret_cast<const uchar2*>(argmax), reinterpret_cast<const uint8_t*>(pass_bits),
      x, dec, batch, channels, H, W / 4, out_shuffle_groups, 1.f / (float)((int64_t)batch * H * W), mean,
      invstd, gamma, dgamma, dbeta, ch_scale, terms, reinterpret_cast<uint4*>(dy_packed), (int64_t)batch * c8n * H * W);
  MNB_LAUNCHED(1);
  return 0;
}

extern "C" int mnb_bn_sign_pool_bwd_pack(const float* g, const uint32_t* pass_bits, const uint8_t* argmax, const float* x,
                                         int32_t batch, int32_t channels, int32_t H, int32_t W, const float* mean,
                                         const float* invstd, const float* gamma, const float* dgamma, const float* dbeta,
                                         int32_t out_shuffle_groups, const float* ch_scale, int32_t terms, void* dy_packed,
                                         mnb_stream_t stream) {
  return bn_sign_pool_bwd_pack<float>(g, pass_bits, argmax, x, nullptr, batch, channels, H, W, mean, invstd, gamma, dgamma, dbeta,
                                      out_shuffle_groups, ch_scale, terms, dy_packed, stream);
}

extern "C" int mnb_bn_sign_pool_bwd_pack_codes(const float* g, const uint32_t* pass_bits, const uint8_t* argmax,
                                               const int16_t* codes, const float* dec, int32_t batch, int32_t channels, int32_t H,
                                               int32_t W, const float* mean, const float* invstd, const float* gamma,
                                               const float* dgamma, const float* dbeta, int32_t out_shuffle_groups,
                                               const float* ch_scale, int32_t terms, void* dy_packed, mnb_stream_t stream) {
  MNB_REQUIRE(dec, "NULL decode pair");
  return bn_sign_pool_bwd_pack<int16_t>(g, pass_bits, argmax, codes, dec, batch, channels, H, W, mean, invstd, gamma, dgamma,
                                        dbeta, out_shuffle_groups, ch_scale, terms, dy_packed, stream);
}

extern "C" int mnb_quant_add_pack_fwd(const float* a, const float* b, int32_t batch, int32_t channels, int32_t h, int32_t w,
                                      const mnb_act_qparams* qp, int32_t relu, float* out, const mnb_pk_post* post,
                                      mnb_stream_t stream) {
  return quant_add_pack<8>(a, b, batch, channels, h, w, qp, relu, out, post, stream);
}

extern "C" int mnb_bn_relu_quant_pack_fwd(const float* x, int32_t batch, int32_t channels, int32_t hw, const float* mean,
                                          const float* invstd, const float* gamma, const float* beta,
                                          const mnb_act_qparams* qp, int32_t out_shuffle_groups, void* x_packed,
                                          uint32_t* pass_bits, mnb_stream_t stream) {
  MNB_REQUIRE(x && mean && invstd && gamma && beta && qp && x_packed && pass_bits, "NULL bn_relu_quant_pack pointer");
  MNB_REQUIRE(batch > 0 && channels > 0 && hw > 0, "bad bn_relu_quant_pack shape");
  MNB_REQUIRE(qp->mode == MNB_ACT_DOREFA && qp->bits >= 2 && qp->bits <= 8, "the fused producer takes a DoReFa quantizer with 2..8 bits");
  MNB_REQUIRE(out_shuffle_groups >= 1 && channels % out_shuffle_groups == 0, "shuffle groups %d do not divide %d channels",
              out_shuffle_groups, channels);
  if (channels % 8 || hw % 32 || (reinterpret_cast<uintptr_t>(x_packed) & 15))
    return mnb_fail(MNB_E_UNSUPPORTED, "fused producer needs channels %% 8 == 0, H*W %% 32 == 0, 16-byte aligned output");
  const int64_t warps = (int64_t)batch * (channels / 8) * (hw / 32);
  const int blocks = (int)std::min<int64_t>(mnb_ceil_div(warps, 8), (int64_t)MNB_NUM_SMS * 16);
  pk::bn_relu_quant_pack_kernel<<<blocks, 256, 0, (cudaStream_t)stream>>>(x, batch, channels, hw, out_shuffle_groups, mean, invstd,
                                                                       gamma, beta, *qp, pass_bits,
                                                                       reinterpret_cast<uint4*>(x_packed));
  MNB_LAUNCHED(1);
  return 0;
}

extern "C" int mnb_pk_conv_plan_ex(const mnb_conv_shape* s, int32_t mode, int32_t terms_a, int32_t terms_w, int32_t* out,
                                   int32_t n) {
  pk::Plan p;
  if (int e = pk::make_plan(s, mode, terms_a, terms_w, p)) return e;
  if (out) plan_fields(p, out, n);
  return 0;
}

extern "C" int mnb_pk_conv_plan(const mnb_conv_shape* s, int32_t mode, int32_t terms_a, int32_t terms_w, int32_t* out16) {
  return mnb_pk_conv_plan_ex(s, mode, terms_a, terms_w, out16, 16);
}

extern "C" int64_t mnb_pk_wimage_bytes(const mnb_conv_shape* s, int32_t mode, int32_t terms_a, int32_t terms_w) {
  pk::Plan p;
  if (pk::make_plan(s, mode, terms_a, terms_w, p)) return -1;
  return p.wimg_bytes;
}

extern "C" int mnb_pk_pack_weight(const mnb_conv_shape* s, int32_t mode, int32_t terms_a, int32_t terms_w,
                                  const int16_t* w_int, const float* w_f32, const float* kzero, void* w_img,
                                  mnb_stream_t stream) {
  MNB_REQUIRE((w_int != nullptr) != (w_f32 != nullptr), "exactly one of w_int / w_f32");
  MNB_REQUIRE(w_img && (reinterpret_cast<uintptr_t>(w_img) & 15) == 0, "weight image must be 16-byte aligned");
  pk::PackWParams pp;
  if (int e = pk::make_plan(s, mode, terms_a, terms_w, pp.pl)) return e;
  pp.w_int = w_int; pp.w_f32 = w_f32; pp.kzero = kzero;
  pp.cin_g = s->in_c / s->groups; pp.cout_g = s->out_c / s->groups;
  const int64_t vecs = pp.pl.wimg_bytes / 16;
  const int blocks = (int)std::min<int64_t>((vecs + 255) / 256, (int64_t)MNB_NUM_SMS * 8);
  pk::pack_weight_kernel<8><<<blocks, 256, 0, (cudaStream_t)stream>>>(pp, reinterpret_cast<uint4*>(w_img));
  MNB_LAUNCHED(1);
  return 0;
}

static int pk_conv_impl(const mnb_conv_shape* s, int32_t mode, const void* a_pk, int32_t terms_a, const void* w_img,
                        int32_t terms_w, const float* n_scale, const float* a_scale, float a_scale_const,
                        const float* bias, const uint8_t* bits8, float gain, float* out, const mnb_pk_post* post,
                        int32_t* err_flag, mnb_stream_t stream, int cpu = 8, int16_t* codes = nullptr, float* dec = nullptr) {
  using namespace pk;
  MNB_REQUIRE(s && a_pk && w_img && (out || post || codes) && err_flag, "NULL pk_conv pointer");
  Plan pl;
  if (int e = make_plan(s, mode, terms_a, terms_w, pl, cpu)) return e;
  if (codes) {
    MNB_REQUIRE(mode == 0 && cpu == 8 && !out && !post && !bits8 && dec, "pk conv: int16 codes are a plain forward output");
    if (pl.segmented || terms_a != 1 || terms_w != 1)
      return unsupported("int16 codes need one activation piece, one weight piece and a non-segmented plan");
  }
  if (post && cpu == 16) {
    MNB_REQUIRE(post->q && post->out_pk && (reinterpret_cast<uintptr_t>(post->out_pk) & 15) == 0, "pk conv: consumer plane / quantizer");
    if (post->q->mode != MNB_ACT_IAO || post->q->q_type != 0 || post->q->bits < 2 || post->q->bits > 8 || post->q->qmin < -128 ||
        post->q->qmax > 127)
      return unsupported("int8 consumer plane needs a symmetric IAO quantizer with 2..8 bits");
    if (pl.G > 1 && (pl.ng % 16)) return unsupported("int8 consumer plane of a grouped conv needs channels per group % 16 == 0");
  }
  if (post) {
    MNB_REQUIRE(mode == 0 && !bits8, "pk conv: a fused consumer is a forward-only (inference) option");
    MNB_REQUIRE(post->q && post->out_pk && (reinterpret_cast<uintptr_t>(post->out_pk) & 15) == 0, "pk conv: consumer plane / quantizer");
    MNB_REQUIRE(post->q->mode == MNB_ACT_DOREFA || post->q->mode == MNB_ACT_IAO, "pk conv: consumer quantizer must be DoReFa or IAO");
    MNB_REQUIRE(post->q->bits >= 2 && post->q->bits <= 8, "pk conv: consumer levels must fit one bf16 piece (2..8 bits)");
    if (pl.G > 1 && (pl.ng % 8)) return unsupported("fused consumer of a grouped conv needs channels per group % 8 == 0");
    if (post->phase_split && ((pl.OH | pl.OW) & 1)) return unsupported("stride-2 consumer of an odd-sized plane");
    if (pl.segmented) return unsupported("fused consumer of a segmented (multi-piece) plan");
  }
  if (bits8 && pl.G > 1 && (pl.ng % 8)) return unsupported("STE mask of a grouped conv needs channels per group % 8 == 0");
  static ConvParams p;
  memset(&p, 0, sizeof(p));
  ConvParams::Mma& m = p.m;
  m.n_items = pl.n_items; m.chunks = pl.chunks; m.ksteps = pl.ksteps; m.MT = pl.MT; m.Nt = pl.Nt; m.npairs = pl.npairs;
  m.st_mask = pl.nstage - 1; m.st_log2 = pl.st_log2; m.stage16 = pl.stage_bytes >> 4;
  m.a_term16 = pl.a_bytes >> 4; m.a_mt16 = (pl.TA * pl.a_bytes) >> 4; m.a_k16 = 2 * pl.npos;
  m.b_off16 = pl.b_off >> 4; m.b_tap16 = (pl.CC / cpu) * pl.Nt; m.b_k16 = 2 * pl.Nt;
  m.a_lbo = (uint32_t)pl.npos * 16u; m.b_lbo = (uint32_t)pl.Nt * 16u;
  m.seg_len = (uint32_t)pl.seg_len;
  int nprog = 0;
  uint32_t* prog = reinterpret_cast<uint32_t*>(m.prog4);
  for (int i = 0; i < MAXPROG; ++i) prog[i] = 0xffffffffu;
  for (int y = 0; y < pl.ny; ++y) {
    m.ntmpl[y] = pl.ntmpl[y]; p.ntmpl[y] = pl.ntmpl[y];
    for (int t = 0; t < pl.ntmpl[y]; ++t) {
      const Tmpl& tp = pl.tmpl[y][t];
      p.tmpl_kph[y][t] = tp.kph; p.tmpl_blk_off[y][t] = tp.blk_off; p.tmpl_blk_bytes[y][t] = tp.blk_bytes;
      const int cnt = tp.ntap * pl.npairs * pl.ksteps;
      nprog = (nprog + 3) & ~3;
      m.tmpl_begin[y][t] = (uint16_t)(nprog / 4); m.tmpl_cnt[y][t] = (uint16_t)((cnt + 3) / 4);
      if (nprog + ((cnt + 3) & ~3) > MAXPROG) return unsupported("MMA program longer than 512 entries");
      for (int pr = 0; pr < pl.npairs; ++pr)
        for (int i = 0; i < tp.ntap; ++i)
          for (int j = 0; j < pl.ksteps; ++j) {
            const uint32_t a16 = (uint32_t)pl.tap_aoff[y][tp.tap0 + i] + (uint32_t)pl.pair_a[pr] * m.a_term16 + (uint32_t)j * m.a_k16;
            const uint32_t b16 = (uint32_t)i * m.b_tap16 + (uint32_t)pl.pair_b[pr] * (uint32_t)tp.ntap * m.b_tap16 + (uint32_t)j * m.b_k16;
            if (a16 > 0xffffu || b16 > 0xffffu) return mnb_fail(MNB_E_ARG, "pk conv: MMA program offset overflow");
            prog[nprog++] = a16 | (b16 << 16);
          }
    }
    p.img_bytes[y] = pl.img_bytes[y]; p.y_off[y] = pl.y_off[y];
  }
  p.n_items = pl.n_items; p.n_ntiles = pl.n_ntiles; p.G = pl.G; p.MT = pl.MT; p.TA = pl.TA; p.chunks = pl.chunks;
  p.CC8 = pl.CC / cpu; p.C8A = pl.C8A; p.kg8 = pl.kg / cpu; p.stage_bytes = pl.stage_bytes; p.a_bytes = pl.a_bytes;
  p.a_box_bytes = pl.a_box_bytes; p.b_off = pl.b_off; p.st_mask = pl.nstage - 1; p.st_log2 = pl.st_log2;
  p.Wt = pl.Wt; p.TH = pl.TH; p.TB = pl.TB; p.wlo = pl.wlo; p.hlo = pl.hlo; p.col_tiles = pl.col_tiles; p.row_tiles = pl.row_tiles;
  p.n_mtiles = pl.n_mtiles;
  p.w_img = reinterpret_cast<const uint8_t*>(w_img);
  p.B = pl.B; p.THH = pl.THH; p.BW = pl.BW; p.OHr = pl.OHr; p.OWr = pl.OWr; p.OH = pl.OH; p.OW = pl.OW; p.omul = pl.omul; p.ny = pl.ny;
  p.ng = pl.ng; p.Nt = pl.Nt; p.NOUT = pl.NOUT; p.C8O = ceil_div(pl.NOUT, cpu); p.smem_bytes = pl.smem_bytes; p.off_stg = pl.off_stg;
  p.mode = mode;
  p.n_scale = n_scale; p.a_scale = a_scale; p.a_scale_const = a_scale_const; p.bias = bias; p.bits8 = bits8; p.gain = gain;
  p.out = out; p.err = err_flag; p.codes = codes; p.dec = dec;
  if (post) {
    p.post_out = reinterpret_cast<uint4*>(post->out_pk); p.post_q = *post->q; p.post_relu = post->relu; p.post_split = post->phase_split;
  }
  { static const int dbg = [] { const char* e = getenv("MNB_PK_DEBUG"); return e ? atoi(e) : 0; }(); p.dbg = dbg; }
  CUtensorMap tm[3];
  const int C8tot = pl.nkph * pl.C8A;
  const int64_t plane_bytes = (int64_t)pl.B * C8tot * pl.HA * pl.WA * 16;
  for (int t = 0; t < 3; ++t) {
    const int tt = t < pl.TA ? t : 0;
    if (int e = make_pk_tmap(&tm[t], a_pk, plane_bytes, tt, pl.B, C8tot, pl.HA, pl.WA, pl.BW, pl.THH, pl.TB, pl.CC / cpu)) return e;
  }
  if (pl.n_items >= (1 << 22) || pl.n_mtiles >= (1 << 22))
    return mnb_fail(MNB_E_UNSUPPORTED, "pk conv: %d work items / %d M tiles exceed the index arithmetic of the kernel", pl.n_items, pl.n_mtiles);
  const int gx = std::max(1, std::min(pl.n_items, MNB_NUM_SMS / pl.ny));
  using ConvFn = void (*)(const CUtensorMap, const CUtensorMap, const CUtensorMap, const ConvParams);
#define MNB_PK_CONV_FNS(SEG, I8) {pk_conv_kernel<SEG, 16, I8>, pk_conv_kernel<SEG, 32, I8>, pk_conv_kernel<SEG, 48, I8>, \
                                  pk_conv_kernel<SEG, 64, I8>, pk_conv_kernel<SEG, 96, I8>, pk_conv_kernel<SEG, 128, I8>}
  static const ConvFn fns[3][6] = {MNB_PK_CONV_FNS(false, false), MNB_PK_CONV_FNS(true, false), MNB_PK_CONV_FNS(false, true)};
#undef MNB_PK_CONV_FNS
  int ki = -1;
  for (int i = 0; i < 6; ++i) if (kNtSizes[i] == pl.Nt) ki = i;
  if (ki < 0 || pl.MT * pl.Nt > 128) return mnb_fail(MNB_E_ARG, "pk conv: plan with Nt %d, MT %d", pl.Nt, pl.MT);
  const ConvFn fn = fns[cpu == 16 ? 2 : (pl.segmented ? 1 : 0)][ki];
  if (int e = set_max_smem(fn, kSmemBudget)) return e;
  fn<<<dim3(gx, pl.ny), kConvThreads, pl.smem_bytes, (cudaStream_t)stream>>>(tm[0], tm[1], tm[2], p);
  MNB_LAUNCHED(1);
  return 0;
}

extern "C" int mnb_pk_conv(const mnb_conv_shape* s, int32_t mode, const void* a_pk, int32_t terms_a, const void* w_img,
                           int32_t terms_w, const float* n_scale, const float* a_scale, float a_scale_const,
                           const float* bias, const uint8_t* bits8, float gain, float* out, int32_t* err_flag,
                           mnb_stream_t stream) {
  MNB_REQUIRE(out, "NULL pk_conv output");
  return pk_conv_impl(s, mode, a_pk, terms_a, w_img, terms_w, n_scale, a_scale, a_scale_const, bias, bits8, gain, out, nullptr,
                      err_flag, stream);
}

extern "C" int mnb_pk_conv_post(const mnb_conv_shape* s, const void* a_pk, int32_t terms_a, const void* w_img, int32_t terms_w,
                                const float* n_scale, const float* a_scale, float a_scale_const, const float* bias,
                                float* out, const mnb_pk_post* post, int32_t* err_flag, mnb_stream_t stream) {
  MNB_REQUIRE(post, "NULL consumer description");
  return pk_conv_impl(s, 0, a_pk, terms_a, w_img, terms_w, n_scale, a_scale, a_scale_const, bias, nullptr, 1.f, out, post,
                      err_flag, stream);
}

extern "C" int mnb_pk_conv_codes(const mnb_conv_shape* s, const void* a_pk, int32_t terms_a, const void* w_img, int32_t terms_w,
                                 const float* n_scale, const float* a_scale, float a_scale_const, const float* bias,
                                 int32_t level_bound, int16_t* codes, float* dec, int32_t* err_flag, mnb_stream_t stream) {
  MNB_REQUIRE(s && codes && dec, "NULL pk_conv_codes pointer");
  MNB_REQUIRE(level_bound >= 1 && s->groups >= 1, "pk_conv_codes: level bound %d", level_bound);
  if ((int64_t)(s->in_c / s->groups) * s->ker_h * s->ker_w * level_bound > 32767)
    return mnb_fail(MNB_E_UNSUPPORTED, "pk_conv_codes: sums of %d x %d x %d terms of level %d may exceed int16", s->in_c / s->groups,
                    s->ker_h, s->ker_w, level_bound);
  return pk_conv_impl(s, 0, a_pk, terms_a, w_img, terms_w, n_scale, a_scale, a_scale_const, bias, nullptr, 1.f, nullptr, nullptr,
                      err_flag, stream, 8, codes, dec);
}


extern "C" int64_t mnb_pk_i8_act_bytes(int32_t batch, int32_t channels, int32_t h, int32_t w) {
  return (int64_t)batch * ((channels + 15) / 16) * h * w * 16;
}

extern "C" int mnb_pk_i8_pack_act(const float* x, int32_t batch, int32_t channels, int32_t h, int32_t w, const mnb_act_qparams* qp,
                                  int32_t phase_split, int32_t relu, void* out_pk, mnb_stream_t stream) {
  MNB_REQUIRE(x && qp && out_pk, "NULL pk_i8_pack_act pointer");
  MNB_REQUIRE(batch > 0 && channels > 0 && h > 0 && w > 0, "bad pk_i8_pack_act arguments");
  MNB_REQUIRE((reinterpret_cast<uintptr_t>(out_pk) & 15) == 0, "packed tensor must be 16-byte aligned");
  if (!i8_quantizer(qp)) return mnb_fail(MNB_E_UNSUPPORTED, "int8 plane needs a symmetric IAO quantizer with 2..8 bits");
  if (phase_split) MNB_REQUIRE(((h | w) & 1) == 0, "phase split needs even H and W");
  MNB_REQUIRE((int64_t)h * w < (1ll << 31), "pk_i8_pack_act: plane too large");
  const int C16 = (channels + 15) / 16;
  dim3 blocks, threads;
  if (!unit_grid(batch, C16, h * w, blocks, threads))
    return mnb_fail(MNB_E_UNSUPPORTED, "pk_i8_pack_act: %d (image, unit) planes exceed the grid", batch * C16);
  pk::pack_act_i8_kernel<<<blocks, threads, 0, (cudaStream_t)stream>>>(x, batch, channels, h, w, C16, *qp, phase_split,
                                                                               relu, reinterpret_cast<uint4*>(out_pk));
  MNB_LAUNCHED(1);
  return 0;
}

extern "C" int mnb_pk_i8_conv_plan(const mnb_conv_shape* s, int32_t* out, int32_t n) {
  pk::Plan p;
  if (int e = pk::make_plan(s, 0, 1, 1, p, 16)) return e;
  if (out) plan_fields(p, out, n);
  return 0;
}

extern "C" int64_t mnb_pk_i8_wimage_bytes(const mnb_conv_shape* s) {
  pk::Plan p;
  if (pk::make_plan(s, 0, 1, 1, p, 16)) return -1;
  return p.wimg_bytes;
}

extern "C" int mnb_pk_i8_pack_weight(const mnb_conv_shape* s, const int16_t* w_int, void* w_img, mnb_stream_t stream) {
  MNB_REQUIRE(w_int, "NULL pk_i8_pack_weight levels");
  MNB_REQUIRE(w_img && (reinterpret_cast<uintptr_t>(w_img) & 15) == 0, "weight image must be 16-byte aligned");
  pk::PackWParams pp;
  if (int e = pk::make_plan(s, 0, 1, 1, pp.pl, 16)) return e;
  pp.w_int = w_int; pp.w_f32 = nullptr; pp.kzero = nullptr;
  pp.cin_g = s->in_c / s->groups; pp.cout_g = s->out_c / s->groups;
  const int64_t vecs = pp.pl.wimg_bytes / 16;
  const int blocks = (int)std::min<int64_t>((vecs + 255) / 256, (int64_t)MNB_NUM_SMS * 8);
  pk::pack_weight_kernel<16><<<blocks, 256, 0, (cudaStream_t)stream>>>(pp, reinterpret_cast<uint4*>(w_img));
  MNB_LAUNCHED(1);
  return 0;
}

extern "C" int mnb_pk_i8_conv(const mnb_conv_shape* s, const void* a_pk, const void* w_img, const float* n_scale,
                              const float* a_scale, float a_scale_const, const float* bias, float* out, const mnb_pk_post* post,
                              int32_t* err_flag, mnb_stream_t stream) {
  MNB_REQUIRE(out || post, "pk_i8_conv: NULL out needs a consumer plane (post)");
  return pk_conv_impl(s, 0, a_pk, 1, w_img, 1, n_scale, a_scale, a_scale_const, bias, nullptr, 1.f, out, post, err_flag, stream, 16);
}

extern "C" int mnb_quant_add_pack_i8_fwd(const float* a, const float* b, int32_t batch, int32_t channels, int32_t h, int32_t w,
                                         const mnb_act_qparams* qp, int32_t relu, float* out, const mnb_pk_post* post,
                                         mnb_stream_t stream) {
  return quant_add_pack<16>(a, b, batch, channels, h, w, qp, relu, out, post, stream);
}

extern "C" int64_t mnb_pk_wgrad_scratch_bytes(const mnb_conv_shape* s, int32_t terms_dy, int32_t terms_x) {
  pk::WgPlan p;
  if (pk::make_wg_plan(s, terms_dy, terms_x, p)) return -1;
  return p.partial_floats * 4;
}

extern "C" int mnb_pk_wgrad_plan(const mnb_conv_shape* s, int32_t terms_dy, int32_t terms_x, int32_t* out, int32_t n) {
  pk::WgPlan p;
  if (int e = pk::make_wg_plan(s, terms_dy, terms_x, p)) return e;
  if (out) {
    const int v[10] = {p.Nc, p.n_ctiles, p.tpg, p.n_tg, p.gm, p.splits, p.NI, p.nstage, p.BW, p.TH};
    for (int i = 0; i < std::min(n, 10); ++i) out[i] = v[i];
  }
  return 0;
}

extern "C" int mnb_pk_wgrad(const mnb_conv_shape* s, const void* dy_pk, int32_t terms_dy, const void* x_pk, int32_t terms_x,
                            const float* a_scale, const float* kdiv, float* dw, void* scratch, int32_t* err_flag,
                            mnb_stream_t stream) {
  using namespace pk;
  MNB_REQUIRE(s && dy_pk && x_pk && dw && scratch && err_flag, "NULL pk_wgrad pointer");
  WgPlan pl;
  if (int e = make_wg_plan(s, terms_dy, terms_x, pl)) return e;
  static WgParams p;
  memset(&p, 0, sizeof(p));
  WgParams::Mma& m = p.m;
  m.stg_per_split = pl.stg_per_split; m.nstg_total = pl.nstg_total; m.NI = pl.NI; m.ksteps = pl.rows_dy / 16; m.ntap = pl.ntap;
  m.Nc = pl.Nc; m.tpg = pl.tpg; m.n_tg = pl.n_tg; m.npairs = pl.npairs; m.st_mask = pl.nstage - 1; m.st_log2 = pl.st_log2; m.stage16 = pl.stage_bytes >> 4;
  m.sub16 = pl.sub_bytes >> 4; m.dy_term16 = pl.dy_bytes >> 4; m.x_off16 = (pl.TA * pl.dy_bytes) >> 4;
  m.x_term16 = (pl.nkph_used * pl.x_bytes) >> 4; m.x_kph16 = pl.x_bytes >> 4;
  m.dy_sbo = (uint32_t)pl.rows_dy * 16u; m.x_sbo = (uint32_t)pl.rows_x * 16u; m.nsub = pl.nsub;
  for (int i = 0; i < pl.npairs; ++i) { m.pair_a16[i] = pl.pair_a[i] * m.dy_term16; m.pair_b16[i] = pl.pair_b[i] * m.x_term16; }
  {
    m.g4 = (uint32_t)ceil_div(pl.tpg, 4);
    if ((size_t)pl.npairs * pl.n_tg * m.g4 > sizeof(m.progb4) / sizeof(uint4)) return unsupported("wgrad issue program too long");
    uint32_t* prog = reinterpret_cast<uint32_t*>(m.progb4);
    for (size_t i = 0; i < sizeof(m.progb4) / 4; ++i) prog[i] = 0xffffffffu;
    for (int i = 0; i < pl.npairs; ++i)
      for (int tg = 0; tg < pl.n_tg; ++tg)
        for (int tt = 0; tt < pl.tpg && tg * pl.tpg + tt < pl.ntap; ++tt) {
          const int t = tg * pl.tpg + tt;
          prog[((size_t)(i * pl.n_tg + tg) * m.g4) * 4 + tt] = m.pair_b16[i] + pl.kph_slot[pl.tap_kph[t]] * m.x_kph16 + pl.tap_off[t];
        }
  }
  p.G = pl.G; p.n_ktiles = pl.n_ktiles; p.n_ctiles = pl.n_ctiles; p.n_tg = pl.n_tg; p.tpg = pl.tpg; p.splits = pl.splits; p.stg_per_split = pl.stg_per_split;
  p.nstg_total = pl.nstg_total; p.NI = pl.NI; p.nsub = pl.nsub; p.row_tiles = pl.row_tiles; p.TA = pl.TA; p.TX = pl.TX;
  p.nkph_used = pl.nkph_used;
  for (int i = 0; i < 4; ++i) p.kph_used[i] = pl.kph_used[i];
  p.K8 = pl.K8; p.C8X = pl.C8X; p.cout_g8 = pl.cout_g / 8; p.cin_g8 = pl.cin_g / 8; p.Nc8 = pl.Nc / 8; p.TH = pl.TH; p.hlo = pl.hlo;
  p.wlo = pl.wlo; p.stage_bytes = pl.stage_bytes; p.sub_bytes = pl.sub_bytes; p.dy_bytes = pl.dy_bytes; p.x_bytes = pl.x_bytes;
  p.dy_box_bytes = pl.dy_box_bytes; p.x_box_bytes = pl.x_box_bytes; p.st_mask = pl.nstage - 1; p.st_log2 = pl.st_log2;
  p.smem_bytes = pl.smem_bytes; p.ntap = pl.ntap; p.Nc = pl.Nc; p.cout_g = pl.cout_g; p.cin_g = pl.cin_g;
  p.partial = reinterpret_cast<float*>(scratch); p.err = err_flag;
  CUtensorMap tdy[3], tx[3];
  const int64_t dy_plane = (int64_t)pl.B * pl.K8 * pl.P * pl.Q * 16;
  const int C8tot = pl.nkph * pl.C8X;
  const int64_t x_plane = (int64_t)pl.B * C8tot * pl.HX * pl.WX * 16;
  for (int t = 0; t < 3; ++t) {
    if (int e = make_pk_tmap(&tdy[t], dy_pk, dy_plane, t < pl.TA ? t : 0, pl.B, pl.K8, pl.P, pl.Q, pl.BW, pl.TH, 1, 16)) return e;
    if (int e = make_pk_tmap(&tx[t], x_pk, x_plane, t < pl.TX ? t : 0, pl.B, C8tot, pl.HX, pl.WX, pl.BW, pl.THH, 1, pl.Nc / 8)) return e;
  }
  using WgFn = void (*)(const CUtensorMap, const CUtensorMap, const CUtensorMap, const CUtensorMap, const CUtensorMap,
                        const CUtensorMap, const WgParams);
  static const WgFn wfns[8] = {pk_wgrad_kernel<16>, pk_wgrad_kernel<32>, pk_wgrad_kernel<48>, pk_wgrad_kernel<64>,
                               pk_wgrad_kernel<80>, pk_wgrad_kernel<96>, pk_wgrad_kernel<112>, pk_wgrad_kernel<128>};
  if (pl.Nc % 16 || pl.Nc < 16 || pl.Nc > 128) return mnb_fail(MNB_E_ARG, "pk wgrad: plan with Nc %d", pl.Nc);
  const WgFn wfn = wfns[pl.Nc / 16 - 1];
  if (int e = set_max_smem(wfn, kSmemBudget)) return e;
  cudaStream_t st = (cudaStream_t)stream;
  wfn<<<dim3(pl.G * pl.n_ktiles * pl.n_ctiles * pl.n_tg, pl.splits), kWgThreads, pl.smem_bytes, st>>>(tdy[0], tdy[1], tdy[2], tx[0],
                                                                                                     tx[1], tx[2], p);
  {
    const int cout_o = pl.cout_g / pl.gm, cin_o = pl.cin_g / pl.gm;
    const dim3 rgrid(cin_o * pl.ntap, (cout_o + 127) / 128, pl.G * pl.gm);
    wg_reduce_kernel<<<rgrid, 128, 0, st>>>(p.partial, pl.splits, pl.G, pl.gm, pl.n_ktiles, pl.n_ctiles, pl.ntap, pl.Nc, cout_o,
                                            cin_o, a_scale, kdiv, dw);
  }
  MNB_LAUNCHED(2);
  return 0;
}

extern "C" int mnb_pk_wgrad_taps_plan(const mnb_conv_shape* s, int32_t terms_dy, int32_t terms_x, int32_t* out, int32_t n) {
  pk::WgPlan p;
  if (int e = pk::make_wgt_plan(s, terms_dy, terms_x, p)) return e;
  if (out) {
    const int64_t sb = p.partial_floats * 4;
    const int v[12] = {p.G, p.splits, p.NI, p.nstage, p.BW, p.TH, p.stg_per_split, p.smem_bytes, pk::kTapsN * 16,
                       (int)(sb & 0x7fffffff), (int)(sb >> 31), p.npairs};
// ... 43 lines not shown
```

### micronet_b200/functional.py

```python
from __future__ import annotations

import ctypes as C

import torch
from torch.autograd import Function

from . import _lib as L


class KernelTimer:

    def __init__(self):
        self.records = []

    def run(self, kind, sh, fn):
        a, b = torch.cuda.Event(enable_timing=True), torch.cuda.Event(enable_timing=True)
        a.record()
        rc = fn()
        b.record()
        self.records.append((kind, tuple(getattr(sh, f) for f, _ in sh._fields_), a, b))
        return rc

    def summary(self):
        out = {}
# ... 135 lines not shown
        L.check(lib.mnb_dorefa_weight_bwd(g.data_ptr(), ctx.aux.data_ptr(), g.numel(), ctx.w_bits,
                                          dw.data_ptr(), L.scratch(g.device).data_ptr(), L.stream()),
                "dorefa_weight_bwd")
        return dw, None


class WbWeightFn(Function):

    @staticmethod
    def forward(ctx, w, W):
        L.require_cuda(w)
        lib = L.load()
        assert w.is_contiguous() and w.dim() == 4
        k, cpg, khw = w.shape[0], w.shape[1], w.shape[2] * w.shape[3]
        wq = torch.empty_like(w)
        w_int = torch.empty(w.shape, dtype=torch.int16, device=w.device)
        w_scale = torch.empty(k, dtype=torch.float32, device=w.device)
        aux = torch.empty(3 * k, dtype=torch.float32, device=w.device)
        L.check(lib.mnb_wb_weight_fwd(w.data_ptr(), k, cpg, khw, W, w_int.data_ptr(), w_scale.data_ptr(),
                                      wq.data_ptr(), aux.data_ptr(), L.stream()), "wb_weight_fwd")
        ctx.w, ctx.aux, ctx.W = w.detach(), aux, W
        ctx.mark_non_differentiable(w_int, w_scale)
        return wq, w_int, w_scale

    @staticmethod
    def backward(ctx, g, _gi, _gs):
        lib = L.load()
        g = g.contiguous()
        w = ctx.w
        dw = torch.empty_like(g)
        L.check(lib.mnb_wb_weight_bwd(g.data_ptr(), w.data_ptr(), ctx.aux.data_ptr(), w.shape[0], w.shape[1],
                                      w.shape[2] * w.shape[3], ctx.W, dw.data_ptr(), L.stream()),
                "wb_weight_bwd")
        return dw, None


class IaoWeightFn(Function):

    @staticmethod
    def forward(ctx, w, scale, zero_point, obs_min, obs_max, q_type, qmin, qmax):
        L.require_cuda(w)
        lib = L.load()
        w = w.contiguous()
        n, k, rows = w.numel(), w.shape[0], scale.numel()
        wq = torch.empty_like(w)
        w_int = torch.empty(w.shape, dtype=torch.int16, device=w.device)
        w_scale = torch.empty(k, dtype=torch.float32, device=w.device)
        keep = torch.empty(w.shape, dtype=torch.uint8, device=w.device)
        L.check(lib.mnb_iao_weight_fwd(w.data_ptr(), n, k, rows, scale.data_ptr(), zero_point.data_ptr(),
                                       obs_min.data_ptr(), obs_max.data_ptr(), q_type, qmin, qmax,
                                       w_int.data_ptr(), w_scale.data_ptr(), wq.data_ptr(), keep.data_ptr(),
                                       L.stream()), "iao_weight_fwd")
        ctx.keep, ctx.scale, ctx.k, ctx.rows = keep, scale, k, rows
        ctx.mark_non_differentiable(w_int, w_scale)
        return wq, w_int, w_scale

    @staticmethod
    def backward(ctx, g, _gi, _gs):
        lib = L.load()
        g = g.contiguous()
        dw = torch.empty_like(g)
        L.check(lib.mnb_iao_weight_bwd(g.data_ptr(), ctx.keep.data_ptr(), ctx.scale.data_ptr(), g.numel(),
                                       ctx.k, ctx.rows, dw.data_ptr(), L.stream()), "iao_weight_bwd")
        return (dw,) + (None,) * 7


def _shape_struct(x_shape, w_shape, stride, padding, dilation, groups):
    b, c, h, w = x_shape
    k, _, r, s = w_shape
    return L.ConvShape(b, c, h, w, k, r, s, stride[0], stride[1], padding[0], padding[1],
                       dilation[0], dilation[1], groups)


def _out_hw(sh: L.ConvShape):
    p = (sh.in_h + 2 * sh.pad_h - sh.dil_h * (sh.ker_h - 1) - 1) // sh.stride_h + 1
    q = (sh.in_w + 2 * sh.pad_w - sh.dil_w * (sh.ker_w - 1) - 1) // sh.stride_w + 1
    return p, q


def channel_sums(x4):
    lib = L.load()
    b, c = x4.shape[0], x4.shape[1]
    hw = x4.numel() // (b * c)
    out = torch.empty(2 * c, dtype=torch.float32, device=x4.device)
    L.check(lib.mnb_channel_stats(x4.data_ptr(), b, c, hw, 0, out.data_ptr(),
                                  L.scratch(x4.device, c).data_ptr(), L.stream()), "channel_stats")
    return out[:c]



def materialized(t):
    codes = getattr(t, "_mnb_codes", None)
    if codes is not None:
        b, c = t.shape[0], t.shape[1]
        out = torch.empty(t.shape, dtype=torch.float32, device=t.device)
        L.check(L.load().mnb_codes_decode(codes[0].data_ptr(), codes[1].data_ptr(), b, c, t.numel() // (b * c), out.data_ptr(),
                                          L.stream()), "codes_decode")
        return out
    if not getattr(t, "_mnb_plane_only", False):
        return t
    b, c, h, w = t.shape
    plane = t._mnb_pk_pm1.view(torch.bfloat16).view(b, c // 8, h, w, 8)
    return plane.permute(0, 1, 4, 2, 3).reshape(b, c, h, w).float()


def xnor_preferred(sh, has_plane):
    return not has_plane


def _pk_terms(spec, w_int, pm1=False):
    T = L.PK_TERMS
    if spec is None:
        ta = 1 if pm1 else T
    else:
        ta = 2 if (spec.mode == L.ACT_IAO and spec.q_type == 1) else 1
    return ta, (1 if w_int is not None else T)


def _pk_forward(ctx, x, wq, bias, w_int, w_scale, spec, sh, y, need_dx, prepacked=None, pre_relu=False, pm1=False,
                codes_out=False):
    from . import pk as PK
    ta, tw = _pk_terms(spec, w_int, pm1)
    if not PK.supported(sh, 0, ta, tw):
        return False
    Tb = min(L.PK_TERMS, L.PK_TERMS_BWD)
    if need_dx and not PK.supported(sh, 1, Tb, 1 if w_int is not None else Tb):
        return False
    if ctx.needs_input_grad[1] and not PK.wgrad_supported(sh, Tb, min(ta, Tb)):
        return False
    qp = spec.struct() if spec is not None else None
    split = sh.stride_h == 2
    if prepacked is not None:
        x_pk, bits8 = prepacked, None
    else:
        x_pk, bits8 = PK.pack_act(x, qp, ta, phase_split=split, want_bits=need_dx, relu=pre_relu)
    src = w_int if w_int is not None else wq
    cache = getattr(src, "_mnb_pk_cache", None)
    ckey = (PK._key(sh), ta, tw)
    w_img = cache.get(ckey) if cache is not None else None
    if w_img is None:
        w_img = PK.pack_weight(sh, 0, ta, tw, w_int=w_int, w_f32=None if w_int is not None else wq)
        if cache is not None:
            cache[ckey] = w_img
    a_scale, a_const = None, 1.0
    if spec is not None:
        if spec.mode == L.ACT_IAO:
            a_scale = spec.scale.clone() if (need_dx or ctx.needs_input_grad[1]) else spec.scale
        elif spec.mode == L.ACT_DOREFA:
            a_const = 1.0 / float(2 ** spec.bits - 1)
    rc = L.E_UNSUPPORTED
    if codes_out and w_int is not None and ta == 1 and tw == 1:
        codes = torch.empty(y.shape, dtype=torch.int16, device=y.device)
        dec = torch.empty(2 * y.shape[1], dtype=torch.float32, device=y.device)
        rc = _timed("fwd_pk", sh, lambda: PK.conv_codes(sh, x_pk, w_img, codes, dec, n_scale=w_scale, a_scale=a_scale,
                                                        a_scale_const=a_const, bias=bias))
        if rc == 0:
            y._mnb_codes = (codes, dec)
    if rc == L.E_UNSUPPORTED:
        rc = _timed("fwd_pk", sh, lambda: PK.conv(sh, 0, x_pk, ta, w_img, tw, y,
                                                  n_scale=w_scale if w_int is not None else None,
                                                  a_scale=a_scale, a_scale_const=a_const, bias=bias))
    if rc == L.E_UNSUPPORTED:
        return False
    L.check(rc, "pk_conv fwd")
    ctx.pk = True
    ctx.pk_x, ctx.pk_ta, ctx.pk_bits8, ctx.pk_a_scale, ctx.pk_prepacked = x_pk, ta, bits8, a_scale, prepacked is not None
    return True


def _pk_backward(ctx, dy):
    from . import pk as PK
    sh, spec = ctx.sh, ctx.spec
    T = min(L.PK_TERMS, L.PK_TERMS_BWD)
    int_w = ctx.w_int is not None
    need_dx, need_dw = ctx.needs_input_grad[0], ctx.needs_input_grad[1]
    fold = int_w and need_dx
    pre = getattr(dy, "_mnb_pk_dy", None)
    if pre is not None:
        if pre[1] != T or (pre[2] is not None) != fold:
            raise RuntimeError("micronet_b200: packed gradient operand does not match this layer's backward configuration")
        dy_pk = pre[0]
    else:
        dy_pk, _ = PK.pack_act(dy, None, T, ch_scale=ctx.w_scale if fold else None)
    dx = dwq = None
    if need_dx:
        tw = 1 if int_w else T
        w_img = PK.pack_weight(sh, 1, T, tw, w_int=ctx.w_int, w_f32=None if int_w else ctx.wq,
                               kzero=ctx.w_scale if int_w else None)
        dx = torch.empty((sh.batch, sh.in_c, sh.in_h, sh.in_w), dtype=torch.float32, device=dy.device)
        gain = 0.1 if (spec is not None and spec.mode == L.ACT_DOREFA) else 1.0
        plain_gain = gain if ctx.pk_prepacked else 1.0
        L.check(_timed("dgrad_pk", sh, lambda: PK.conv(sh, 1, dy_pk, T, w_img, tw, dx, bits8=ctx.pk_bits8, gain=gain,
                                                       a_scale_const=plain_gain)), "pk_conv dgrad")
    if need_dw:
        dwq = torch.empty_like(ctx.wq)
        a_scale = None
        if spec is not None:
            a_scale = ctx.pk_a_scale if spec.mode == L.ACT_IAO else _dorefa_scale_tensor(spec.bits, dy.device)
        tx = min(ctx.pk_ta, T)
        kdiv = ctx.w_scale if fold else None
        fn = PK.wgrad_taps if L.PK_WG_TAPS and PK.wgrad_taps_plan(sh, T, tx) is not None else PK.wgrad
        L.check(_timed("wgrad_pk", sh, lambda: fn(sh, dy_pk, T, ctx.pk_x, tx, dwq, a_scale=a_scale, kdiv=kdiv)), "pk_wgrad")
    return dx, dwq


class QuantConv2dFn(Function):

    @staticmethod
    def forward(ctx, x, wq, bias, w_int, w_scale, spec, stride, padding, dilation, groups, pre_relu=False, no_grad=False,
                codes_out=False):
        L.require_cuda(x, wq)
        assert not (pre_relu and any(ctx.needs_input_grad)), "the folded ReLU is an inference-only fusion"
        lib = L.load()
        packed = getattr(x, "_mnb_packed", None) if L.USE_PACKED else None
        x = x.contiguous()
        wq = wq.contiguous()
        sh = _shape_struct(x.shape, wq.shape, stride, padding, dilation, groups)
        p, q = _out_hw(sh)
        y = torch.empty((x.shape[0], wq.shape[0], p, q), dtype=torch.float32, device=x.device)
        codes = bits = None
        a_scale = None
        if spec is not None and spec.mode != L.ACT_SIGN:
            a_scale = spec.scale if spec.mode == L.ACT_IAO else _dorefa_scale_tensor(spec.bits, x.device)
        done = False
        ctx.pk = False
        if (L.XNOR_MODE != "off" and spec is None and w_int is not None and getattr(x, "_mnb_pm1", False)
                and (no_grad or not any(ctx.needs_input_grad[:3])) and x.dtype == torch.float32 and not pre_relu):
            from . import xnor as XN
            if XN.supported(sh) and (L.XNOR_MODE == "all" or xnor_preferred(sh, getattr(x, "_mnb_pk_pm1", None) is not None)):
                a_bits = XN.pack_act(materialized(x), groups)
                rc = _timed("fwd_xnor", sh, lambda: XN.conv(sh, a_bits, XN.pack_weight(sh, w_int), y, alpha=w_scale, bias=bias))
                if rc == 0:
                    done = True
                elif rc != L.E_UNSUPPORTED:
                    L.check(rc, "xnor_conv_fwd")
        pkq = getattr(x, "_mnb_pk_q", None)
        if pkq is not None and not done:
            if spec is None or spec.mode != L.ACT_DOREFA or spec.bits != pkq[1] or w_int is None:
                raise RuntimeError("micronet_b200: a fused producer's packed output reached a conv with another quantizer")
            done = _pk_forward(ctx, x, wq, bias, w_int, w_scale, spec, sh, y, ctx.needs_input_grad[0], prepacked=pkq[0])
            if not done:
                raise RuntimeError("micronet_b200: fused producer output in front of a conv outside the packed-operand cover")
        if (not done and L.PK_MODE != "off" and x.dtype == torch.float32 and (L.PK_MODE == "all" or spec is not None)
                and not getattr(x, "_mnb_plane_only", False)):
            done = _pk_forward(ctx, x, wq, bias, w_int, w_scale, spec, sh, y, ctx.needs_input_grad[0], pre_relu=pre_relu)
        pm1_plane = getattr(x, "_mnb_pk_pm1", None)
        if (not done and L.PK_WBWTAB and L.PK_MODE != "off" and spec is None and w_int is not None and x.dtype == torch.float32
                and getattr(x, "_mnb_pm1", False) and (pm1_plane is not None or sh.ker_h * sh.ker_w > 1)):
            if pm1_plane is not None and pm1_plane.numel() != x.numel() * 2:
                pm1_plane = None
            done = _pk_forward(ctx, x, wq, bias, w_int, w_scale, None, sh, y, ctx.needs_input_grad[0], prepacked=pm1_plane,
                               pm1=True, codes_out=codes_out)
        if (not done and L.PK_MODE != "off" and spec is None and w_int is None and x.dtype == torch.float32
                and getattr(x, "_mnb_pm1", False) and not pre_relu):
            plane = pm1_plane if (pm1_plane is not None and pm1_plane.numel() == x.numel() * 2) else None
            done = _pk_forward(ctx, x, wq, bias, None, None, None, sh, y, ctx.needs_input_grad[0], prepacked=plane, pm1=True)
        if not done and getattr(x, "_mnb_plane_only", False):
            x = materialized(x)
        if not done and pre_relu:
            x = torch.relu(x)
        if not done and packed is not None and spec is None and w_int is not None and packed.numel() == x.numel() \
                and L.PK_MODE != "off" and sh.stride_h == 1:
            from . import pk as PK
            if PK.supported(sh, 0, 1, 1):
                w_img = PK.pack_weight(sh, 0, 1, 1, w_int=w_int)
                rc = _timed("fwd_pk", sh, lambda: PK.conv(sh, 0, packed, 1, w_img, 1, y, n_scale=w_scale, bias=bias))
                if rc == 0:
                    done = True
                elif rc != L.E_UNSUPPORTED:
                    L.check(rc, "pk_conv fwd (packed producer)")
        if not done and L.USE_TC and w_int is not None and x.dtype == torch.float32:
            qp = None
            if spec is not None:
                qp = spec.struct()
                codes = torch.empty(x.shape, dtype=torch.uint8, device=x.device)
                if ctx.needs_input_grad[0]:
                    bits = torch.zeros((x.numel() + 31) // 32, dtype=torch.int32, device=x.device)
            wpack = torch.empty(w_int.numel(), dtype=torch.int16, device=x.device)
            rc = _timed("fwd_tc", sh, lambda: lib.mnb_fq_conv2d_fwd_tc(
                C.byref(sh), x.data_ptr(), None if qp is None else C.byref(qp), w_int.data_ptr(),
                w_scale.data_ptr(), L.ptr(bias), y.data_ptr(), L.ptr(codes), L.ptr(bits), wpack.data_ptr(),
                L.tc_err_flag(x.device).data_ptr(), L.stream()))
            if rc == 0:
                done = True
            elif rc == L.E_UNSUPPORTED:
                codes = bits = None
            else:
                L.check(rc, "fq_conv2d_fwd_tc")
        ctx.fconv = False
        if not done and L.USE_TC and spec is None and x.dtype == torch.float32:
            rc = _timed("fconv_fwd_tc", sh, lambda: lib.mnb_fconv2d_fwd_tc(
                C.byref(sh), x.data_ptr(), wq.data_ptr(), L.ptr(bias), y.data_ptr(),
                L.tc_err_flag(x.device).data_ptr(), L.stream()))
            if rc == 0:
                done = ctx.fconv = True
            elif rc != L.E_UNSUPPORTED:
                L.check(rc, "fconv2d_fwd_tc")
        if not done and L.PK_MODE != "off" and x.dtype == torch.float32:
            done = _pk_forward(ctx, x, wq, bias, w_int, w_scale, spec, sh, y, ctx.needs_input_grad[0])
        if not done:
            ops = L.ConvOperands()
            if spec is not None:
                codes, bits, _ = act_quant_raw(x, spec, True, ctx.needs_input_grad[0], False)
                ops.a_codes = codes.data_ptr()
                ops.a_offset = spec.code_offset
                ops.a_offset_zp = L.ptr(spec.zero_point) if spec.mode == L.ACT_IAO else None
                ops.a_scale = L.ptr(a_scale)
            else:
                ops.a_f32 = x.data_ptr()
            if codes is not None and w_int is not None:
                ops.w_int, ops.w_scale = w_int.data_ptr(), w_scale.data_ptr()
            else:
                ops.w_f32 = wq.data_ptr()
            ops.bias = L.ptr(bias)
            L.check(_timed("fwd", sh, lambda: lib.mnb_conv2d_fwd(C.byref(sh), C.byref(ops), y.data_ptr(), L.stream())),
                    "conv2d_fwd")
        if spec is not None and not ctx.pk and (ctx.needs_input_grad[0] or ctx.needs_input_grad[1]):
            spec = spec.frozen()
            if spec.mode == L.ACT_IAO:
                a_scale = spec.scale
        ctx.sh, ctx.spec, ctx.a_scale = sh, spec, a_scale
        ctx.codes, ctx.bits = codes, bits
        ctx.x = x if (not ctx.pk and (codes is None or (L.USE_TC and w_int is not None))) else None
        ctx.wq = wq
        ctx.w_int, ctx.w_scale = (w_int, w_scale) if w_int is not None else (None, None)
        ctx.has_bias = bias is not None
        if ctx.pk and spec is None and w_int is not None and ctx.needs_input_grad[1]:
            y._mnb_pk_conv = (w_scale if ctx.needs_input_grad[0] else None, min(L.PK_TERMS, L.PK_TERMS_BWD))
        return y

    @staticmethod
    def backward(ctx, dy):
        lib = L.load()
        presummed = getattr(dy, "_mnb_channel_sum", None)
        dy = dy.contiguous()
        sh, spec = ctx.sh, ctx.spec
        dx = dwq = db = None
        if ctx.has_bias and ctx.needs_input_grad[2]:
            db = presummed if presummed is not None and presummed.numel() == dy.shape[1] else channel_sums(dy)
        if ctx.pk:
            dx, dwq = _pk_backward(ctx, dy)
            return dx, dwq, db, None, None, None, None, None, None, None, None, None, None
        if ctx.needs_input_grad[0]:
            dx = torch.empty((sh.batch, sh.in_c, sh.in_h, sh.in_w), dtype=torch.float32, device=dy.device)
            qp = spec.struct() if spec is not None else None
            bits_ptr = ctx.bits.data_ptr() if spec is not None else None
# ... 376 lines not shown
```

### micronet_b200/pk.py

```python
from __future__ import annotations

import ctypes as C

import torch

from . import _lib as L

_plan_cache = {}


def _key(sh):
    return tuple(getattr(sh, f) for f, _ in sh._fields_)


def supported(sh, mode, terms_a, terms_w):
    k = ("c", _key(sh), mode, terms_a, terms_w)
    if k not in _plan_cache:
        _plan_cache[k] = L.load().mnb_pk_conv_plan(C.byref(sh), mode, terms_a, terms_w, None) == 0
    return _plan_cache[k]


def segmented(sh, mode, terms_a, terms_w):
    k = ("s", _key(sh), mode, terms_a, terms_w)
    if k not in _plan_cache:
        out = (C.c_int32 * 17)()
        _plan_cache[k] = L.load().mnb_pk_conv_plan_ex(C.byref(sh), mode, terms_a, terms_w, out, 17) == 0 and out[16] != 0
    return _plan_cache[k]


def wgrad_supported(sh, terms_dy, terms_x):
    k = ("w", _key(sh), terms_dy, terms_x)
    if k not in _plan_cache:
        _plan_cache[k] = int(L.load().mnb_pk_wgrad_scratch_bytes(C.byref(sh), terms_dy, terms_x))
    return _plan_cache[k] >= 0


def pack_act(x, qp, terms, ch_scale=None, phase_split=False, want_bits=False, relu=False):
    lib = L.load()
    b, c, h, w = x.shape
    nbytes = int(lib.mnb_pk_act_bytes(b, c, h, w, terms))
    out = torch.empty(nbytes, dtype=torch.uint8, device=x.device)
    bits = None
    if qp is not None and want_bits:
        bits = torch.empty((b, (c + 7) // 8, h, w), dtype=torch.uint8, device=x.device)
    L.check(lib.mnb_pk_pack_act_relu(x.data_ptr(), b, c, h, w, None if qp is None else C.byref(qp), terms, L.ptr(ch_scale),
                                     1 if phase_split else 0, 1 if relu else 0, out.data_ptr(), L.ptr(bits), L.stream()),
            "pk_pack_act")
    return out, bits


def pack_weight(sh, mode, terms_a, terms_w, w_int=None, w_f32=None, kzero=None):
    lib = L.load()
    nbytes = int(lib.mnb_pk_wimage_bytes(C.byref(sh), mode, terms_a, terms_w))
    if nbytes < 0:
        raise ValueError("micronet_b200.pk: shape outside the cover of the packed-operand convolution")
    dev = (w_int if w_int is not None else w_f32).device
    img = torch.empty(nbytes, dtype=torch.uint8, device=dev)
    L.check(lib.mnb_pk_pack_weight(C.byref(sh), mode, terms_a, terms_w, L.ptr(w_int), L.ptr(w_f32), L.ptr(kzero),
                                   img.data_ptr(), L.stream()), "pk_pack_weight")
    return img


def conv(sh, mode, a_pk, terms_a, w_img, terms_w, out, n_scale=None, a_scale=None, a_scale_const=1.0, bias=None,
         bits8=None, gain=1.0):
    lib = L.load()
    return lib.mnb_pk_conv(C.byref(sh), mode, a_pk.data_ptr(), terms_a, w_img.data_ptr(), terms_w, L.ptr(n_scale),
                           L.ptr(a_scale), float(a_scale_const), L.ptr(bias), L.ptr(bits8), float(gain), out.data_ptr(),
                           L.tc_err_flag(out.device).data_ptr(), L.stream())


def conv_codes(sh, a_pk, w_img, codes, dec, n_scale=None, a_scale=None, a_scale_const=1.0, bias=None, level_bound=1):
    return L.load().mnb_pk_conv_codes(C.byref(sh), a_pk.data_ptr(), 1, w_img.data_ptr(), 1, L.ptr(n_scale), L.ptr(a_scale),
                                      float(a_scale_const), L.ptr(bias), int(level_bound), codes.data_ptr(), dec.data_ptr(),
                                      L.tc_err_flag(codes.device).data_ptr(), L.stream())


def codes_fit(in_channels, groups, kernel_size, level_bound=1):
    r, s = (kernel_size, kernel_size) if isinstance(kernel_size, int) else kernel_size
    return (in_channels // groups) * r * s * level_bound <= 32767


def consumer_plane(b, c, h, w, device):
    return torch.empty(int(L.load().mnb_pk_act_bytes(b, c, h, w, 1)), dtype=torch.uint8, device=device)


def conv_post(sh, a_pk, terms_a, w_img, terms_w, out, post_qp, post_plane, post_relu, post_split, n_scale=None, a_scale=None,
              a_scale_const=1.0, bias=None):
    lib = L.load()
    post = L.PkPost(C.pointer(post_qp), 1 if post_relu else 0, 1 if post_split else 0, post_plane.data_ptr())
    return lib.mnb_pk_conv_post(C.byref(sh), a_pk.data_ptr(), terms_a, w_img.data_ptr(), terms_w, L.ptr(n_scale), L.ptr(a_scale),
                                float(a_scale_const), L.ptr(bias), L.ptr(out), C.byref(post),
                                L.tc_err_flag(a_pk.device).data_ptr(), L.stream())


def i8_plan(sh):
    out = (C.c_int32 * 21)()
    return list(out) if L.load().mnb_pk_i8_conv_plan(C.byref(sh), out, 21) == 0 else None


def i8_supported(sh):
    k = ("i8", _key(sh))
    if k not in _plan_cache:
        _plan_cache[k] = L.load().mnb_pk_i8_conv_plan(C.byref(sh), None, 0) == 0
    return _plan_cache[k]


def consumer_plane_i8(b, c, h, w, device):
    return torch.empty(int(L.load().mnb_pk_i8_act_bytes(b, c, h, w)), dtype=torch.uint8, device=device)


def pack_act_i8(x, qp, phase_split=False, relu=False):
    b, c, h, w = x.shape
    out = consumer_plane_i8(b, c, h, w, x.device)
    L.check(L.load().mnb_pk_i8_pack_act(x.data_ptr(), b, c, h, w, C.byref(qp), 1 if phase_split else 0, 1 if relu else 0,
                                        out.data_ptr(), L.stream()), "pk_i8_pack_act")
    return out


def pack_weight_i8(sh, w_int):
    nbytes = int(L.load().mnb_pk_i8_wimage_bytes(C.byref(sh)))
    if nbytes < 0:
        raise ValueError("micronet_b200.pk: shape outside the cover of the int8 convolution")
    img = torch.empty(nbytes, dtype=torch.uint8, device=w_int.device)
    L.check(L.load().mnb_pk_i8_pack_weight(C.byref(sh), w_int.data_ptr(), img.data_ptr(), L.stream()), "pk_i8_pack_weight")
    return img


def conv_i8(sh, a_pk, w_img, out, n_scale=None, a_scale=None, a_scale_const=1.0, bias=None, post=None):
    pp = None
    if post is not None:
        qp, plane, relu, split = post
        pp = C.byref(L.PkPost(C.pointer(qp), 1 if relu else 0, 1 if split else 0, plane.data_ptr()))
    return L.load().mnb_pk_i8_conv(C.byref(sh), a_pk.data_ptr(), w_img.data_ptr(), L.ptr(n_scale), L.ptr(a_scale),
                                   float(a_scale_const), L.ptr(bias), L.ptr(out), pp, L.tc_err_flag(a_pk.device).data_ptr(),
                                   L.stream())


def wgrad(sh, dy_pk, terms_dy, x_pk, terms_x, dw, a_scale=None, kdiv=None):
    lib = L.load()
    nbytes = int(lib.mnb_pk_wgrad_scratch_bytes(C.byref(sh), terms_dy, terms_x))
    if nbytes < 0:
        return L.E_UNSUPPORTED
    ws = torch.empty(max(nbytes, 16), dtype=torch.uint8, device=dw.device)
    return lib.mnb_pk_wgrad(C.byref(sh), dy_pk.data_ptr(), terms_dy, x_pk.data_ptr(), terms_x, L.ptr(a_scale),
                            L.ptr(kdiv), dw.data_ptr(), ws.data_ptr(), L.tc_err_flag(dw.device).data_ptr(), L.stream())


def wgrad_taps_plan(sh, terms_dy, terms_x):
    k = ("wt", _key(sh), terms_dy, terms_x)
    if k not in _plan_cache:
        out = (C.c_int32 * 12)()
        ok = L.load().mnb_pk_wgrad_taps_plan(C.byref(sh), terms_dy, terms_x, out, 12) == 0
        names = ("blocks", "splits", "NI", "nstage", "BW", "TH", "stg_per_split", "smem_bytes", "acc_regs")
        plan = None
        if ok:
            plan = dict(zip(names, out[:9]))
            plan["scratch_bytes"] = out[9] | (out[10] << 31)
            plan["npairs"] = out[11]
        _plan_cache[k] = plan
    return _plan_cache[k]


def wgrad_taps(sh, dy_pk, terms_dy, x_pk, terms_x, dw, a_scale=None, kdiv=None):
    plan = wgrad_taps_plan(sh, terms_dy, terms_x)
    if plan is None:
        return L.E_UNSUPPORTED
    ws = torch.empty(plan["scratch_bytes"], dtype=torch.uint8, device=dw.device)
    return L.load().mnb_pk_wgrad_taps(C.byref(sh), dy_pk.data_ptr(), terms_dy, x_pk.data_ptr(), terms_x, L.ptr(a_scale),
                                      L.ptr(kdiv), dw.data_ptr(), ws.data_ptr(), L.tc_err_flag(dw.device).data_ptr(), L.stream())
```

Before: 35880.

## Add warp-specialized taps conv kernel for grouped 3x3 convs with two consumer warpgroups

Adds a new persistent tensor-core convolution kernel for grouped 3x3 stride-1 convolutions with 16 input and 32 output channels per group. One producer warp streams activation tiles and weight blocks through an mbarrier ring, while two consumer warpgroups each take alternate work items with a smaller accumulator budget. The forward (codes and float) and data-gradient paths use it by default when the plan matches the existing conv's stages. The goal is better SM occupancy and overlap for these narrow grouped layers. The risks are lower per-warpgroup tile reuse and shapes that fall back to the old path, for example when an STE mask is present.

```diff
diff --git a/harness/conv_taps_probe.py b/harness/conv_taps_probe.py
--- /dev/null
+++ b/harness/conv_taps_probe.py
@@ -0,0 +1,124 @@
+import argparse
+import json
+import os
+import subprocess
+import sys
+
+sys.path.insert(0, os.path.dirname(os.path.dirname(os.path.abspath(__file__))))
+
+SHAPES = {"g16 256->512 @16": (256, 256, 16, 16, 512, 16), "g32 512->1024 @8": (256, 512, 8, 8, 1024, 32)}
+
+
+def card():
+    try:
+        return subprocess.run(["nvidia-smi", "--query-gpu=name,power.limit,clocks.max.sm", "--format=csv,noheader"],
+                              capture_output=True, text=True, timeout=30).stdout.strip().splitlines()[0]
+    except (OSError, subprocess.SubprocessError, IndexError) as e:
+        return f"unknown ({type(e).__name__})"
+
+
+def floor_us(B, Cc, H, W, K, mode):
+    n_in, n_out = B * Cc * H * W, B * K * H * W
+    byts = n_in * 2 + n_out * 2 if mode == "fwd" else n_out * 2 * 2 + n_in * 4
+    return byts / 3.35e12 * 1e6, byts
+
+
+def one_process(args):
+    import torch
+    from micronet_b200 import _lib as L, pk as PK
+    dev = torch.device("cuda:0")
+    have_new = hasattr(PK, "conv_taps")
+    res = {}
+    for name, (B, Cc, H, W, K, G) in SHAPES.items():
+        sh = L.ConvShape(B, Cc, H, W, K, 3, 3, 1, 1, 1, 1, 1, 1, G)
+        g = torch.Generator().manual_seed(11)
+        w_int = torch.randint(-1, 2, (K, Cc // G, 3, 3), generator=g).to(torch.int16).to(dev)
+        w_scale = (torch.rand(K, generator=g) + 0.5).to(dev)
+        wf = PK.pack_weight(sh, 0, 1, 1, w_int=w_int)
+        wd = PK.pack_weight(sh, 1, 2, 1, w_int=w_int, kzero=w_scale)
+        ops = []
+        for _ in range(4):
+            x = torch.randint(0, 2, (B, Cc, H, W), generator=g).float().mul_(2).sub_(1).to(dev)
+            dy = torch.randn(B, K, H, W, generator=g).to(dev)
+            ops.append((PK.pack_act(x, None, 1)[0], PK.pack_act(dy, None, 2, ch_scale=w_scale)[0]))
+        codes = {k: torch.empty(B, K, H, W, dtype=torch.int16, device=dev) for k in ("old", "new")}
+        dec = {k: torch.empty(2 * K, device=dev) for k in ("old", "new")}
+        dx = {k: torch.empty(B, Cc, H, W, device=dev) for k in ("old", "new")}
+
+        def launch(kind, mode, i):
+            x_pk, dy_pk = ops[i % 4]
+            if mode == "fwd":
+                if kind == "old":
+                    return PK.conv_codes(sh, x_pk, wf, codes[kind], dec[kind], n_scale=w_scale, a_scale_const=1.0)
+                return PK.conv_taps_codes(sh, x_pk, wf, codes[kind], dec[kind], n_scale=w_scale, a_scale_const=1.0)
+            if kind == "old":
+                return PK.conv(sh, 1, dy_pk, 2, wd, 1, dx[kind], a_scale_const=0.1)
+            return PK.conv_taps(sh, 1, dy_pk, 2, wd, 1, dx[kind], a_scale_const=0.1)
+
+        kinds = ["old", "new"] if have_new else ["old"]
+        for mode in ("fwd", "dgrad"):
+            def window(kind):
+                a, b = torch.cuda.Event(enable_timing=True), torch.cuda.Event(enable_timing=True)
+                a.record()
+                for i in range(args.iters):
+                    L.check(launch(kind, mode, i), f"{kind} {mode}")
+                b.record()
+                torch.cuda.synchronize()
+                return a.elapsed_time(b) * 1e3 / args.iters
+
+            for k in kinds:
+                window(k)
+            t = {k: [] for k in kinds}
+            for _ in range(args.rounds):
+                for k in kinds:
+                    t[k].append(window(k))
+            L.tc_check()
+            fl, byts = floor_us(B, Cc, H, W, K, mode)
+            r = {"floor_us": round(fl, 1), "bytes": byts}
+            for k in kinds:
+                r[f"{k}_us"] = round(sorted(t[k])[len(t[k]) // 2], 1)
+                r[f"{k}_windows_us"] = [round(v, 1) for v in t[k]]
+            if have_new and args.dbg_value == 0:
+                for k in kinds:
+                    L.check(launch(k, mode, 0), k)
+                torch.cuda.synchronize()
+                if mode == "fwd":
+                    r["identical"] = bool(torch.equal(codes["old"], codes["new"]) and torch.equal(dec["old"], dec["new"]))
+                else:
+                    r["identical"] = bool(torch.equal(dx["old"].view(torch.int32), dx["new"].view(torch.int32)))
+            res[f"{name} {mode}"] = r
+    return res
+
+
+def main():
+    ap = argparse.ArgumentParser()
+    ap.add_argument("--iters", type=int, default=60)
+    ap.add_argument("--rounds", type=int, default=5)
+    ap.add_argument("--dbg", default="0,1,2,8,16")
+    ap.add_argument("--out", default=None)
+    ap.add_argument("--dbg-value", type=int, default=None, help=argparse.SUPPRESS)
+    args = ap.parse_args()
+    if args.dbg_value is not None:
+        print(json.dumps(one_process(args)))
+        return
+    out = {"card": card(), "runs": {}}
+    for d in [int(v) for v in args.dbg.split(",")]:
+        env = dict(os.environ, MNB_PK_DEBUG=str(d))
+        cmd = [sys.executable, "-m", "harness.conv_taps_probe", "--iters", str(args.iters), "--rounds", str(args.rounds),
+               "--dbg-value", str(d)]
+        cp = subprocess.run(cmd, env=env, capture_output=True, text=True,
+                            cwd=os.path.dirname(os.path.dirname(os.path.abspath(__file__))))
+        if cp.returncode != 0:
+            out["runs"][str(d)] = {"error": cp.stderr[-2000:]}
+            continue
+        out["runs"][str(d)] = json.loads(cp.stdout.strip().splitlines()[-1])
+    text = json.dumps(out, indent=1)
+    print(text)
+    if args.out:
+        os.makedirs(args.out, exist_ok=True)
+        with open(os.path.join(args.out, "conv_taps_probe.json"), "w") as f:
+            f.write(text)
+
+
+if __name__ == "__main__":
+    main()
diff --git a/include/micronet_b200.h b/include/micronet_b200.h
--- a/include/micronet_b200.h
+++ b/include/micronet_b200.h
@@ -172,6 +172,11 @@
 int mnb_pk_conv_codes(const mnb_conv_shape* s, const void* a_pk, int32_t terms_a, const void* w_img, int32_t terms_w,
                       const float* n_scale, const float* a_scale, float a_scale_const, const float* bias, int32_t level_bound,
                       int16_t* codes, float* dec, int32_t* err_flag, mnb_stream_t stream);
+int mnb_pk_conv_taps_plan(const mnb_conv_shape* s, int32_t mode, int32_t terms_a, int32_t terms_w, int32_t* out, int32_t n);
+int mnb_pk_conv_taps(const mnb_conv_shape* s, int32_t mode, const void* a_pk, int32_t terms_a, const void* w_img,
+                     int32_t terms_w, const float* n_scale, const float* a_scale, float a_scale_const, const float* bias,
+                     const uint8_t* bits8, float* out, int16_t* codes, float* dec, int32_t level_bound, int32_t* err_flag,
+                     mnb_stream_t stream);
 int mnb_codes_decode(const int16_t* codes, const float* dec, int32_t batch, int32_t channels, int32_t hw, float* x,
                      mnb_stream_t stream);
 int mnb_bn_batch_stats_codes(const int16_t* codes, const float* dec, int32_t batch, int32_t channels, int32_t hw, double eps,
diff --git a/micronet_b200/_lib.py b/micronet_b200/_lib.py
--- a/micronet_b200/_lib.py
+++ b/micronet_b200/_lib.py
@@ -93,6 +93,8 @@
     "mnb_bn_sign_pool_bwd_pack": (C.c_int, [_P, _P, _P, _P, _I, _I, _I, _I, _P, _P, _P, _P, _P, _I, _P, _I, _P, _P]),
     "mnb_pk_conv_post": (C.c_int, [_SHAPE, _P, _I, _P, _I, _P, _P, C.c_float, _P, _P, C.POINTER(PkPost), _P, _P]),
     "mnb_pk_conv_codes": (C.c_int, [_SHAPE, _P, _I, _P, _I, _P, _P, C.c_float, _P, _I, _P, _P, _P, _P]),
+    "mnb_pk_conv_taps_plan": (C.c_int, [_SHAPE, _I, _I, _I, _P, _I]),
+    "mnb_pk_conv_taps": (C.c_int, [_SHAPE, _I, _P, _I, _P, _I, _P, _P, C.c_float, _P, _P, _P, _P, _P, _I, _P, _P]),
     "mnb_codes_decode": (C.c_int, [_P, _P, _I, _I, _I, _P, _P]),
     "mnb_bn_batch_stats_codes": (C.c_int, [_P, _P, _I, _I, _I, _D, _D, _P, _P, _P, _P, _P, _P]),
     "mnb_bn_sign_fwd_packed_codes": (C.c_int, [_P, _P, _I, _I, _I, _P, _P, _P, _P, _I, _P, _P, _P, _P]),
@@ -204,6 +206,7 @@
 PK_TERMS_BWD = int(os.environ.get("MNB_PK_TERMS_BWD", "2"))
 PK_WBWTAB = os.environ.get("MNB_PK_WBWTAB", "1") == "1"
 PK_WG_TAPS = os.environ.get("MNB_PK_WG_TAPS", "1") != "0"
+PK_CONV_TAPS = os.environ.get("MNB_PK_CONV_TAPS", "1") != "0"
 
 XNOR_MODE = os.environ.get("MNB_XNOR", "auto")
 
diff --git a/micronet_b200/csrc/mnb_pk.cu b/micronet_b200/csrc/mnb_pk.cu
--- a/micronet_b200/csrc/mnb_pk.cu
+++ b/micronet_b200/csrc/mnb_pk.cu
@@ -55,7 +55,7 @@
 
 static int unsupported(const char* why) { return mnb_fail(MNB_E_UNSUPPORTED, "pk conv: %s", why); }
 
-static int make_plan(const mnb_conv_shape* s, int mode, int TA, int TBk, Plan& p, int cpu = 8) {
+static int make_plan(const mnb_conv_shape* s, int mode, int TA, int TBk, Plan& p, int cpu = 8, int acc_cap = 128) {
   MNB_REQUIRE(s != nullptr, "conv shape is NULL");
   memset(&p, 0, sizeof(p));
   const int C = s->in_c, K = s->out_c, G = s->groups, H = s->in_h, W = s->in_w, R = s->ker_h, S = s->ker_w;
@@ -181,7 +181,7 @@
       const int64_t ctas = std::max<int64_t>(1, MNB_NUM_SMS / p.ny);
       return (double)items / (double)(ceil_div((int)std::min<int64_t>(items, 1 << 30), (int)ctas) * ctas);
     };
-    const int cap = std::max(1, 128 / p.Nt);
+    const int cap = std::max(1, acc_cap / p.Nt);
     for (int mt = 2; mt <= std::min(4, cap); mt *= 2) {
       if (p.n_mtiles < mt) break;
       if ((int64_t)ceil_div(p.n_mtiles, mt) * p.n_ntiles * G * p.ny < 120) break;
@@ -190,7 +190,7 @@
   }
   if (const char* e = getenv("MNB_PK_MT")) {
     const int v = atoi(e);
-    if ((v == 1 || v == 2 || v == 4) && v * p.Nt <= 128) p.MT = v;
+    if ((v == 1 || v == 2 || v == 4) && v * p.Nt <= acc_cap) p.MT = v;
   }
   p.n_mgroups = ceil_div(p.n_mtiles, p.MT);
   p.n_items = p.n_mgroups * p.n_ntiles * G;
@@ -259,7 +259,7 @@
   p.st_log2 = p.nstage == 8 ? 3 : (p.nstage == 4 ? 2 : 1);
   p.off_stg = p.nstage * p.stage_bytes + slack;
   p.smem_bytes = p.off_stg + stg;
-  if (p.MT * p.Nt > 128) return unsupported("accumulators exceed the register budget");
+  if (p.MT * p.Nt > acc_cap) return unsupported("accumulators exceed the register budget");
   return 0;
 }
 
@@ -985,6 +985,179 @@
         }
       }
       epi_bar_sync<NEPI>();
+    }
+  }
+done:
+  __syncthreads();
+}
+
+constexpr int kTapsAcc = 64;
+
+struct alignas(16) TapsShared {
+  uint64_t full[MAXST], empty[MAXST];
+  uint32_t abort;
+  alignas(16) float epi_scale[2][64];
+  alignas(16) float epi_bias[2][64];
+};
+
+__device__ __forceinline__ void wg_bar_sync(int id) { asm volatile("bar.sync %0, 128;" ::"r"(id) : "memory"); }
+
+template <int NT>
+__global__ void __launch_bounds__(kConvThreads, 1)
+pk_conv_taps_kernel(const __grid_constant__ CUtensorMap tmap0, const __grid_constant__ CUtensorMap tmap1,
+                    const __grid_constant__ ConvParams p) {
+  extern __shared__ __align__(1024) uint8_t smem[];
+  __shared__ TapsShared sh;
+  const int tid = threadIdx.x, warp = tid >> 5, lane = tid & 31;
+
+  if (tid == 0) {
+    for (int i = 0; i < MAXST; ++i) { tc::mbar_init(&sh.full[i], 1); tc::mbar_init(&sh.empty[i], 4); }
+    sh.abort = 0;
+    tc::fence_barrier_init();
+    tc::prefetch_tmap(&tmap0);
+    if (p.TA > 1) tc::prefetch_tmap(&tmap1);
+  }
+  for (int i = tid; i < p.smem_bytes / 16; i += kConvThreads) reinterpret_cast<uint4*>(smem)[i] = make_uint4(0, 0, 0, 0);
+  tc::fence_proxy_async_smem();
+  __syncthreads();
+
+  if (warp == 0) {
+    if (lane == 0) {
+      uint32_t sc = 0;
+      const FastDiv d_nt(p.n_ntiles), d_g(p.G), d_ct(p.col_tiles), d_rt(p.row_tiles);
+      for (int it = blockIdx.x; it < p.n_items; it += gridDim.x) {
+        uint32_t nt, r1, g, mg;
+        d_nt.divmod((uint32_t)it, r1, nt);
+        d_g.divmod(r1, mg, g);
+        const uint8_t* wsrc = p.w_img + (size_t)(nt * p.G + g) * (size_t)p.img_bytes[0];
+        for (int t = 0; t < p.ntmpl[0]; ++t) {
+          const uint32_t blk = (uint32_t)p.tmpl_blk_bytes[0][t];
+          const uint8_t* bsrc = wsrc + p.tmpl_blk_off[0][t];
+          for (int cc = 0; cc < p.chunks; ++cc, ++sc) {
+            const uint32_t slot = sc & (uint32_t)p.st_mask, ph = (sc >> p.st_log2) & 1u;
+            if (!tc::mbar_wait(&sh.empty[slot], ph ^ 1u, p.err, 721)) goto done;
+            const bool ld_a = !(p.dbg & 8), ld_b = !(p.dbg & 16);
+            tc::mbar_arrive_expect_tx(&sh.full[slot], (ld_a ? (uint32_t)(p.MT * p.TA * p.a_box_bytes) : 0u) + (ld_b ? blk : 0u));
+            uint8_t* sbase = smem + (size_t)slot * p.stage_bytes;
+            const int c8 = g * p.kg8 + cc * p.CC8;
+            for (int mt = 0; mt < (ld_a ? p.MT : 0); ++mt) {
+              const uint32_t tile = mg * (uint32_t)p.MT + (uint32_t)mt;
+              uint32_t ct, r2, rt, bt;
+              d_ct.divmod(tile, r2, ct);
+              d_rt.divmod(r2, bt, rt);
+              const int cw = (int)ct * p.Wt - p.wlo, chh = (int)rt * p.TH - p.hlo, cb = (int)bt * p.TB;
+              tc::tma_load_4d(sbase + (size_t)(mt * p.TA) * p.a_bytes, &tmap0, &sh.full[slot], 2 * cw, chh, cb, c8);
+              if (p.TA > 1) tc::tma_load_4d(sbase + (size_t)(mt * p.TA + 1) * p.a_bytes, &tmap1, &sh.full[slot], 2 * cw, chh, cb, c8);
+            }
+            if (ld_b) tc::bulk_load_1d(sbase + p.b_off, bsrc + (size_t)cc * blk, blk, &sh.full[slot]);
+          }
+        }
+      }
+    }
+  } else if (warp >= 4) {
+    constexpr int NR = NT / 2, MAXMT = kTapsAcc / NT;
+    const int wg = (warp - 4) >> 2, et = (tid - 128) & 127;
+    float* stage = reinterpret_cast<float*>(smem + p.off_stg) + wg * 16 * tc::kStageLd;
+    float* epi_sc = sh.epi_scale[wg];
+    float* epi_bs = sh.epi_bias[wg];
+    const int tb = et / (p.THH * p.BW);
+    const int rem = et - tb * (p.THH * p.BW);
+    const int th = rem / p.BW, wc = rem - th * p.BW;
+    const bool row_ok = tb < p.TB && th < p.TH && wc < p.Wt;
+    const int64_t plane = (int64_t)p.OH * p.OW;
+    const float a_sc = p.a_scale ? __ldg(p.a_scale) : p.a_scale_const;
+    const uint64_t a_desc0 = tc::smem_desc_kmajor_noswz(tc::smem_u32(smem), p.m.a_lbo, 128);
+    const uint64_t b_desc0 = tc::smem_desc_kmajor_noswz(tc::smem_u32(smem), p.m.b_lbo, 128) + (uint64_t)p.m.b_off16;
+    const uint32_t a_lo0 = (uint32_t)a_desc0, b_lo0 = (uint32_t)b_desc0;
+    const uint64_t a_hi = a_desc0 & 0xffffffff00000000ull, b_hi = b_desc0 & 0xffffffff00000000ull;
+    const uint32_t spi = p.m.ntmpl[0] * p.m.chunks;
+    const FastDiv e_nt(p.n_ntiles), e_g(p.G), e_ct(p.col_tiles), e_rt(p.row_tiles);
+    int k = wg;
+    for (int it = blockIdx.x + wg * gridDim.x; it < p.n_items; it += 2 * gridDim.x, k += 2) {
+      uint32_t nt_u, r1_u, g_u, mg_u;
+      e_nt.divmod((uint32_t)it, r1_u, nt_u);
+      e_g.divmod(r1_u, mg_u, g_u);
+      const int nt = (int)nt_u, mg = (int)mg_u;
+      const int n_base = (int)g_u * p.ng + nt * p.Nt;
+      const int n_cnt = min(p.Nt, p.ng - nt * p.Nt);
+      const bool has_n = et < n_cnt;
+      const float nsc = has_n && p.n_scale ? __ldg(p.n_scale + n_base + et) : 1.f;
+      const float nbs = has_n && p.bias ? __ldg(p.bias + n_base + et) : 0.f;
+      float acc[MAXMT][2][NR];
+#pragma unroll
+      for (int mt = 0; mt < MAXMT; ++mt) { tc::zero_acc(acc[mt][0]); tc::zero_acc(acc[mt][1]); }
+      uint32_t sc = (uint32_t)k * spi;
+      for (uint32_t t = 0; t < p.m.ntmpl[0]; ++t) {
+        const uint32_t pb = p.m.tmpl_begin[0][t], pc = p.m.tmpl_cnt[0][t];
+        for (uint32_t cc = 0; cc < p.m.chunks; ++cc, ++sc) {
+          const uint32_t slot = sc & p.m.st_mask, ph = (sc >> p.m.st_log2) & 1u;
+          tc::mbar_wait_soft(&sh.full[slot], ph, p.err, 723, &sh.abort);
+          const uint32_t s16 = slot * p.m.stage16;
+          tc::wg_fence();
+#pragma unroll
+          for (int mt = 0; mt < MAXMT; ++mt) { tc::fence_acc(acc[mt][0]); tc::fence_acc(acc[mt][1]); }
+          if (!(p.dbg & 2)) {
+#pragma unroll
+            for (int mt = 0; mt < MAXMT; ++mt) {
+              if (mt >= (int)p.m.MT) break;
+              const uint32_t a_base = a_lo0 + s16 + (uint32_t)mt * p.m.a_mt16, b_base = b_lo0 + s16;
+              for (uint32_t e = 0; e < pc; ++e) {
+                const uint4 w4 = p.m.prog4[pb + e];
+                const uint32_t w[4] = {w4.x, w4.y, w4.z, w4.w};
+#pragma unroll
+                for (int q = 0; q < 4; ++q) {
+                  if (w[q] == 0xffffffffu) continue;
+                  const uint64_t bd = b_hi | (uint64_t)(b_base + (w[q] >> 16));
+                  tc::Mma<NT>::template bf16<0, 0>(acc[mt][0], a_hi | (uint64_t)(a_base + (w[q] & 0xffffu)), bd, 1);
+                  tc::Mma<NT>::template bf16<0, 0>(acc[mt][1], a_hi | (uint64_t)(a_base + 64u + (w[q] & 0xffffu)), bd, 1);
+                }
+              }
+            }
+          }
+          tc::wg_commit();
+          tc::wg_wait<0>();
+#pragma unroll
+          for (int mt = 0; mt < MAXMT; ++mt) { tc::fence_acc(acc[mt][0]); tc::fence_acc(acc[mt][1]); }
+          __syncwarp();
+          if (lane == 0) tc::mbar_arrive(&sh.empty[slot]);
+        }
+      }
+      if (et < p.Nt) {
+        const float scv = has_n ? (p.n_scale ? __fmul_rn(a_sc, nsc) : a_sc) : 1.f;
+        epi_sc[et] = scv; epi_bs[et] = nbs;
+        if (p.dec && mg == 0 && has_n) { p.dec[n_base + et] = scv; p.dec[p.NOUT + n_base + et] = nbs; }
+      }
+      const int ncols = (int)p.m.MT * NT;
+#pragma unroll
+      for (int rnd = 0; rnd < MAXMT * NT / 16; ++rnd) {
+        if (16 * rnd >= ncols) break;
+        const int mt = 16 * rnd / NT, n0 = 16 * rnd % NT;
+        wg_bar_sync(1 + wg);
+        tc::frag_cols_to_smem(acc[mt][0], stage, tc::kStageLd, 0, n0, 16);
+        tc::frag_cols_to_smem(acc[mt][1], stage, tc::kStageLd, 64, n0, 16);
+        wg_bar_sync(1 + wg);
+        const int tile = mg * p.MT + mt;
+        uint32_t ct_u, r2_u, rt_u, bt_u;
+        e_ct.divmod((uint32_t)tile, r2_u, ct_u);
+        e_rt.divmod(r2_u, bt_u, rt_u);
+        const int b = (int)bt_u * p.TB + tb, i = (int)rt_u * p.TH + th, j = (int)ct_u * p.Wt + wc;
+        const bool valid = row_ok && tile < p.n_mtiles && b < p.B && i < p.OHr && j < p.OWr;
+        if (!valid || n0 >= n_cnt || (p.dbg & 1)) continue;
+        const int64_t o = ((int64_t)b * p.NOUT + n_base + n0) * plane + (int64_t)i * p.OW + j;
+        const float* sr = stage + et;
+        if (p.codes) {
+          int16_t* cp = p.codes + o;
+#pragma unroll
+          for (int q = 0; q < 16; ++q, cp += plane)
+            if (n0 + q < n_cnt) *cp = (int16_t)__float2int_rn(sr[q * tc::kStageLd]);
+        } else {
+          float* op = p.out + o;
+#pragma unroll
+          for (int q = 0; q < 16; ++q, op += plane)
+            if (n0 + q < n_cnt) *op = fmaf(sr[q * tc::kStageLd], epi_sc[n0 + q], epi_bs[n0 + q]);
+        }
+      }
+      wg_bar_sync(1 + wg);
     }
   }
 done:
@@ -1671,37 +1844,9 @@
   return 0;
 }
 
-static int pk_conv_impl(const mnb_conv_shape* s, int32_t mode, const void* a_pk, int32_t terms_a, const void* w_img,
-                        int32_t terms_w, const float* n_scale, const float* a_scale, float a_scale_const,
-                        const float* bias, const uint8_t* bits8, float gain, float* out, const mnb_pk_post* post,
-                        int32_t* err_flag, mnb_stream_t stream, int cpu = 8, int16_t* codes = nullptr, float* dec = nullptr) {
+static int conv_params(const pk::Plan& pl, int mode, int cpu, const void* a_pk, const void* w_img, pk::ConvParams& p,
+                       CUtensorMap (&tm)[3]) {
   using namespace pk;
-  MNB_REQUIRE(s && a_pk && w_img && (out || post || codes) && err_flag, "NULL pk_conv pointer");
-  Plan pl;
-  if (int e = make_plan(s, mode, terms_a, terms_w, pl, cpu)) return e;
-  if (codes) {
-    MNB_REQUIRE(mode == 0 && cpu == 8 && !out && !post && !bits8 && dec, "pk conv: int16 codes are a plain forward output");
-    if (pl.segmented || terms_a != 1 || terms_w != 1)
-      return unsupported("int16 codes need one activation piece, one weight piece and a non-segmented plan");
-  }
-  if (post && cpu == 16) {
-    MNB_REQUIRE(post->q && post->out_pk && (reinterpret_cast<uintptr_t>(post->out_pk) & 15) == 0, "pk conv: consumer plane / quantizer");
-    if (post->q->mode != MNB_ACT_IAO || post->q->q_type != 0 || post->q->bits < 2 || post->q->bits > 8 || post->q->qmin < -128 ||
-        post->q->qmax > 127)
-      return unsupported("int8 consumer plane needs a symmetric IAO quantizer with 2..8 bits");
-    if (pl.G > 1 && (pl.ng % 16)) return unsupported("int8 consumer plane of a grouped conv needs channels per group % 16 == 0");
-  }
-  if (post) {
-    MNB_REQUIRE(mode == 0 && !bits8, "pk conv: a fused consumer is a forward-only (inference) option");
-    MNB_REQUIRE(post->q && post->out_pk && (reinterpret_cast<uintptr_t>(post->out_pk) & 15) == 0, "pk conv: consumer plane / quantizer");
-    MNB_REQUIRE(post->q->mode == MNB_ACT_DOREFA || post->q->mode == MNB_ACT_IAO, "pk conv: consumer quantizer must be DoReFa or IAO");
-    MNB_REQUIRE(post->q->bits >= 2 && post->q->bits <= 8, "pk conv: consumer levels must fit one bf16 piece (2..8 bits)");
-    if (pl.G > 1 && (pl.ng % 8)) return unsupported("fused consumer of a grouped conv needs channels per group % 8 == 0");
-    if (post->phase_split && ((pl.OH | pl.OW) & 1)) return unsupported("stride-2 consumer of an odd-sized plane");
-    if (pl.segmented) return unsupported("fused consumer of a segmented (multi-piece) plan");
-  }
-  if (bits8 && pl.G > 1 && (pl.ng % 8)) return unsupported("STE mask of a grouped conv needs channels per group % 8 == 0");
-  static ConvParams p;
   memset(&p, 0, sizeof(p));
   ConvParams::Mma& m = p.m;
   m.n_items = pl.n_items; m.chunks = pl.chunks; m.ksteps = pl.ksteps; m.MT = pl.MT; m.Nt = pl.Nt; m.npairs = pl.npairs;
@@ -1742,13 +1887,7 @@
   p.B = pl.B; p.THH = pl.THH; p.BW = pl.BW; p.OHr = pl.OHr; p.OWr = pl.OWr; p.OH = pl.OH; p.OW = pl.OW; p.omul = pl.omul; p.ny = pl.ny;
   p.ng = pl.ng; p.Nt = pl.Nt; p.NOUT = pl.NOUT; p.C8O = ceil_div(pl.NOUT, cpu); p.smem_bytes = pl.smem_bytes; p.off_stg = pl.off_stg;
   p.mode = mode;
-  p.n_scale = n_scale; p.a_scale = a_scale; p.a_scale_const = a_scale_const; p.bias = bias; p.bits8 = bits8; p.gain = gain;
-  p.out = out; p.err = err_flag; p.codes = codes; p.dec = dec;
-  if (post) {
-    p.post_out = reinterpret_cast<uint4*>(post->out_pk); p.post_q = *post->q; p.post_relu = post->relu; p.post_split = post->phase_split;
-  }
   { static const int dbg = [] { const char* e = getenv("MNB_PK_DEBUG"); return e ? atoi(e) : 0; }(); p.dbg = dbg; }
-  CUtensorMap tm[3];
   const int C8tot = pl.nkph * pl.C8A;
   const int64_t plane_bytes = (int64_t)pl.B * C8tot * pl.HA * pl.WA * 16;
   for (int t = 0; t < 3; ++t) {
@@ -1757,6 +1896,47 @@
   }
   if (pl.n_items >= (1 << 22) || pl.n_mtiles >= (1 << 22))
     return mnb_fail(MNB_E_UNSUPPORTED, "pk conv: %d work items / %d M tiles exceed the index arithmetic of the kernel", pl.n_items, pl.n_mtiles);
+  return 0;
+}
+
+static int pk_conv_impl(const mnb_conv_shape* s, int32_t mode, const void* a_pk, int32_t terms_a, const void* w_img,
+                        int32_t terms_w, const float* n_scale, const float* a_scale, float a_scale_const,
+                        const float* bias, const uint8_t* bits8, float gain, float* out, const mnb_pk_post* post,
+                        int32_t* err_flag, mnb_stream_t stream, int cpu = 8, int16_t* codes = nullptr, float* dec = nullptr) {
+  using namespace pk;
+  MNB_REQUIRE(s && a_pk && w_img && (out || post || codes) && err_flag, "NULL pk_conv pointer");
+  Plan pl;
+  if (int e = make_plan(s, mode, terms_a, terms_w, pl, cpu)) return e;
+  if (codes) {
+    MNB_REQUIRE(mode == 0 && cpu == 8 && !out && !post && !bits8 && dec, "pk conv: int16 codes are a plain forward output");
+    if (pl.segmented || terms_a != 1 || terms_w != 1)
+      return unsupported("int16 codes need one activation piece, one weight piece and a non-segmented plan");
+  }
+  if (post && cpu == 16) {
+    MNB_REQUIRE(post->q && post->out_pk && (reinterpret_cast<uintptr_t>(post->out_pk) & 15) == 0, "pk conv: consumer plane / quantizer");
+    if (post->q->mode != MNB_ACT_IAO || post->q->q_type != 0 || post->q->bits < 2 || post->q->bits > 8 || post->q->qmin < -128 ||
+        post->q->qmax > 127)
+      return unsupported("int8 consumer plane needs a symmetric IAO quantizer with 2..8 bits");
+    if (pl.G > 1 && (pl.ng % 16)) return unsupported("int8 consumer plane of a grouped conv needs channels per group % 16 == 0");
+  }
+  if (post) {
+    MNB_REQUIRE(mode == 0 && !bits8, "pk conv: a fused consumer is a forward-only (inference) option");
+    MNB_REQUIRE(post->q && post->out_pk && (reinterpret_cast<uintptr_t>(post->out_pk) & 15) == 0, "pk conv: consumer plane / quantizer");
+    MNB_REQUIRE(post->q->mode == MNB_ACT_DOREFA || post->q->mode == MNB_ACT_IAO, "pk conv: consumer quantizer must be DoReFa or IAO");
+    MNB_REQUIRE(post->q->bits >= 2 && post->q->bits <= 8, "pk conv: consumer levels must fit one bf16 piece (2..8 bits)");
+    if (pl.G > 1 && (pl.ng % 8)) return unsupported("fused consumer of a grouped conv needs channels per group % 8 == 0");
+    if (post->phase_split && ((pl.OH | pl.OW) & 1)) return unsupported("stride-2 consumer of an odd-sized plane");
+    if (pl.segmented) return unsupported("fused consumer of a segmented (multi-piece) plan");
+  }
+  if (bits8 && pl.G > 1 && (pl.ng % 8)) return unsupported("STE mask of a grouped conv needs channels per group % 8 == 0");
+  static ConvParams p;
+  CUtensorMap tm[3];
+  if (int e = conv_params(pl, mode, cpu, a_pk, w_img, p, tm)) return e;
+  p.n_scale = n_scale; p.a_scale = a_scale; p.a_scale_const = a_scale_const; p.bias = bias; p.bits8 = bits8; p.gain = gain;
+  p.out = out; p.err = err_flag; p.codes = codes; p.dec = dec;
+  if (post) {
+    p.post_out = reinterpret_cast<uint4*>(post->out_pk); p.post_q = *post->q; p.post_relu = post->relu; p.post_split = post->phase_split;
+  }
   const int gx = std::max(1, std::min(pl.n_items, MNB_NUM_SMS / pl.ny));
   using ConvFn = void (*)(const CUtensorMap, const CUtensorMap, const CUtensorMap, const ConvParams);
 #define MNB_PK_CONV_FNS(SEG, I8) {pk_conv_kernel<SEG, 16, I8>, pk_conv_kernel<SEG, 32, I8>, pk_conv_kernel<SEG, 48, I8>, \
@@ -1800,6 +1980,67 @@
                     s->ker_h, s->ker_w, level_bound);
   return pk_conv_impl(s, 0, a_pk, terms_a, w_img, terms_w, n_scale, a_scale, a_scale_const, bias, nullptr, 1.f, nullptr, nullptr,
                       err_flag, stream, 8, codes, dec);
+}
+
+
+static int make_taps_plan(const mnb_conv_shape* s, int mode, int TA, int TBk, pk::Plan& p) {
+  using namespace pk;
+  MNB_REQUIRE(s != nullptr, "conv shape is NULL");
+  MNB_REQUIRE(mode == 0 || mode == 1, "pk conv taps: mode %d", mode);
+  const int G = s->groups;
+  if (G < 1 || s->in_c % G || s->out_c % G) return unsupported("taps: bad grouping");
+  if (s->ker_h != 3 || s->ker_w != 3 || s->stride_h != 1 || s->stride_w != 1 || s->pad_h != 1 || s->pad_w != 1 ||
+      s->dil_h != 1 || s->dil_w != 1)
+    return unsupported("taps: 3x3 filters, stride 1, padding 1, dilation 1 only");
+  if (s->in_c / G != 16 || s->out_c / G != 32 || G % 4)
+    return unsupported("taps: 16 input and 32 output channels per group, groups %% 4 == 0 only");
+  if (TBk != 1) return unsupported("taps: one weight piece only");
+  if (mode == 0 ? TA != 1 : (TA < 1 || TA > 2)) return unsupported("taps: forward on one piece, data gradient on one or two");
+  Plan g;
+  if (int e = make_plan(s, mode, TA, TBk, g)) return e;
+  if (int e = make_plan(s, mode, TA, TBk, p, 8, kTapsAcc)) return e;
+  bool same = !g.segmented && !p.segmented && p.ny == 1 && p.Nt == g.Nt && p.n_ntiles == g.n_ntiles && p.CC == g.CC &&
+              p.ksteps == g.ksteps && p.chunks == g.chunks && p.ntmpl[0] == g.ntmpl[0] && p.wimg_bytes == g.wimg_bytes &&
+              (p.Nt == 16 || p.Nt == 32);
+  for (int t = 0; same && t < p.ntmpl[0]; ++t)
+    same = memcmp(&p.tmpl[0][t], &g.tmpl[0][t], sizeof(Tmpl)) == 0;
+  if (!same) return unsupported("taps: the plan's stages differ from mnb_pk_conv's");
+  return 0;
+}
+
+extern "C" int mnb_pk_conv_taps_plan(const mnb_conv_shape* s, int32_t mode, int32_t terms_a, int32_t terms_w, int32_t* out,
+                                     int32_t n) {
+  pk::Plan p;
+  if (int e = make_taps_plan(s, mode, terms_a, terms_w, p)) return e;
+  if (out) plan_fields(p, out, n);
+  return 0;
+}
+
+extern "C" int mnb_pk_conv_taps(const mnb_conv_shape* s, int32_t mode, const void* a_pk, int32_t terms_a, const void* w_img,
+                                int32_t terms_w, const float* n_scale, const float* a_scale, float a_scale_const,
+                                const float* bias, const uint8_t* bits8, float* out, int16_t* codes, float* dec,
+                                int32_t level_bound, int32_t* err_flag, mnb_stream_t stream) {
+  using namespace pk;
+  MNB_REQUIRE(s && a_pk && w_img && err_flag, "NULL pk_conv_taps pointer");
+  MNB_REQUIRE((out != nullptr) != (codes != nullptr), "pk_conv_taps: exactly one of out / codes");
+  MNB_REQUIRE(!codes || (mode == 0 && dec && level_bound >= 1), "pk_conv_taps: int16 codes are a forward output with a decode pair");
+  Plan pl;
+  if (int e = make_taps_plan(s, mode, terms_a, terms_w, pl)) return e;
+  if (bits8) return unsupported("taps: no STE mask in the data-gradient epilogue");
+  if (codes && (int64_t)(s->in_c / s->groups) * s->ker_h * s->ker_w * level_bound > 32767)
+    return unsupported("taps: int16 codes of these sums may overflow");
+  static ConvParams p;
+  CUtensorMap tm[3];
+  if (int e = conv_params(pl, mode, 8, a_pk, w_img, p, tm)) return e;
+  p.n_scale = n_scale; p.a_scale = a_scale; p.a_scale_const = a_scale_const; p.bias = bias; p.gain = 1.f;
+  p.out = out; p.err = err_flag; p.codes = codes; p.dec = dec;
+  using TapsFn = void (*)(const CUtensorMap, const CUtensorMap, const ConvParams);
+  const TapsFn fn = pl.Nt == 16 ? pk_conv_taps_kernel<16> : pk_conv_taps_kernel<32>;
+  if (int e = set_max_smem(fn, kSmemBudget)) return e;
+  const int gx = std::max(1, std::min(pl.n_items, MNB_NUM_SMS));
+  fn<<<gx, kConvThreads, pl.smem_bytes, (cudaStream_t)stream>>>(tm[0], tm[1], p);
+  MNB_LAUNCHED(1);
+  return 0;
 }
 
 
diff --git a/micronet_b200/functional.py b/micronet_b200/functional.py
--- a/micronet_b200/functional.py
+++ b/micronet_b200/functional.py
@@ -311,14 +311,15 @@
     if codes_out and w_int is not None and ta == 1 and tw == 1:
         codes = torch.empty(y.shape, dtype=torch.int16, device=y.device)
         dec = torch.empty(2 * y.shape[1], dtype=torch.float32, device=y.device)
-        rc = _timed("fwd_pk", sh, lambda: PK.conv_codes(sh, x_pk, w_img, codes, dec, n_scale=w_scale, a_scale=a_scale,
-                                                        a_scale_const=a_const, bias=bias))
+        fn = PK.conv_taps_codes if L.PK_CONV_TAPS and PK.conv_taps_plan(sh, 0, 1, 1) is not None else PK.conv_codes
+        rc = _timed("fwd_pk", sh, lambda: fn(sh, x_pk, w_img, codes, dec, n_scale=w_scale, a_scale=a_scale,
+                                             a_scale_const=a_const, bias=bias))
         if rc == 0:
             y._mnb_codes = (codes, dec)
     if rc == L.E_UNSUPPORTED:
-        rc = _timed("fwd_pk", sh, lambda: PK.conv(sh, 0, x_pk, ta, w_img, tw, y,
-                                                  n_scale=w_scale if w_int is not None else None,
-                                                  a_scale=a_scale, a_scale_const=a_const, bias=bias))
+        fn = PK.conv_taps if L.PK_CONV_TAPS and PK.conv_taps_plan(sh, 0, ta, tw) is not None else PK.conv
+        rc = _timed("fwd_pk", sh, lambda: fn(sh, 0, x_pk, ta, w_img, tw, y, n_scale=w_scale if w_int is not None else None,
+                                             a_scale=a_scale, a_scale_const=a_const, bias=bias))
     if rc == L.E_UNSUPPORTED:
         return False
     L.check(rc, "pk_conv fwd")
@@ -349,8 +350,12 @@
         dx = torch.empty((sh.batch, sh.in_c, sh.in_h, sh.in_w), dtype=torch.float32, device=dy.device)
         gain = 0.1 if (spec is not None and spec.mode == L.ACT_DOREFA) else 1.0
         plain_gain = gain if ctx.pk_prepacked else 1.0
-        L.check(_timed("dgrad_pk", sh, lambda: PK.conv(sh, 1, dy_pk, T, w_img, tw, dx, bits8=ctx.pk_bits8, gain=gain,
-                                                       a_scale_const=plain_gain)), "pk_conv dgrad")
+        if L.PK_CONV_TAPS and ctx.pk_bits8 is None and PK.conv_taps_plan(sh, 1, T, tw) is not None:
+            rc = _timed("dgrad_pk", sh, lambda: PK.conv_taps(sh, 1, dy_pk, T, w_img, tw, dx, a_scale_const=plain_gain))
+        else:
+            rc = _timed("dgrad_pk", sh, lambda: PK.conv(sh, 1, dy_pk, T, w_img, tw, dx, bits8=ctx.pk_bits8, gain=gain,
+                                                        a_scale_const=plain_gain))
+        L.check(rc, "pk_conv dgrad")
     if need_dw:
         dwq = torch.empty_like(ctx.wq)
         a_scale = None
diff --git a/micronet_b200/pk.py b/micronet_b200/pk.py
--- a/micronet_b200/pk.py
+++ b/micronet_b200/pk.py
@@ -73,6 +73,28 @@
     return L.load().mnb_pk_conv_codes(C.byref(sh), a_pk.data_ptr(), 1, w_img.data_ptr(), 1, L.ptr(n_scale), L.ptr(a_scale),
                                       float(a_scale_const), L.ptr(bias), int(level_bound), codes.data_ptr(), dec.data_ptr(),
                                       L.tc_err_flag(codes.device).data_ptr(), L.stream())
+
+
+def conv_taps_plan(sh, mode, terms_a, terms_w):
+    k = ("ct", _key(sh), mode, terms_a, terms_w)
+    if k not in _plan_cache:
+        out = (C.c_int32 * 21)()
+        _plan_cache[k] = list(out) if L.load().mnb_pk_conv_taps_plan(C.byref(sh), mode, terms_a, terms_w, out, 21) == 0 else None
+    return _plan_cache[k]
+
+
+def conv_taps(sh, mode, a_pk, terms_a, w_img, terms_w, out, n_scale=None, a_scale=None, a_scale_const=1.0, bias=None,
+              bits8=None):
+    return L.load().mnb_pk_conv_taps(C.byref(sh), mode, a_pk.data_ptr(), terms_a, w_img.data_ptr(), terms_w, L.ptr(n_scale),
+                                     L.ptr(a_scale), float(a_scale_const), L.ptr(bias), L.ptr(bits8), out.data_ptr(), None,
+                                     None, 1, L.tc_err_flag(out.device).data_ptr(), L.stream())
+
+
+def conv_taps_codes(sh, a_pk, w_img, codes, dec, n_scale=None, a_scale=None, a_scale_const=1.0, bias=None, level_bound=1,
+                    terms_a=1):
+    return L.load().mnb_pk_conv_taps(C.byref(sh), 0, a_pk.data_ptr(), terms_a, w_img.data_ptr(), 1, L.ptr(n_scale),
+                                     L.ptr(a_scale), float(a_scale_const), L.ptr(bias), None, None, codes.data_ptr(),
+                                     dec.data_ptr(), int(level_bound), L.tc_err_flag(codes.device).data_ptr(), L.stream())
 
 
 def codes_fit(in_channels, groups, kernel_size, level_bound=1):
```

New measurement: 36610 (median of 6 runs). 2.0% higher.
